# sp-uhh/audio-visual-vad

Hardware: NVIDIA B200
Metric: AV-VAD frames/sec (device-timed) (higher is better)
Workload: dtype bf16

## Files before the change

### audio-visual-vad_b200/csrc/conv_block.cuh

```cuda
#pragma once
#include "conv_slab.cuh"

namespace avvad {
namespace tc {

constexpr int kBlkThreads = 320;
constexpr int kBlkW = 17, kBlkWp = 19;
constexpr int kBlkRows = kBlkWp * kBlkWp;
constexpr uint32_t kBlkSlabBytes = 47104;
constexpr uint32_t kBlkWTile = 32 * 128;
constexpr uint32_t kBlkWBytes = 9 * kBlkWTile;
constexpr uint32_t kBlkOffY = kBlkSlabBytes;
constexpr uint32_t kBlkOffW = 3 * kBlkSlabBytes;
constexpr uint32_t kBlkOffBias = kBlkOffW + 2 * kBlkWBytes;
constexpr uint32_t kBlkOffBar = kBlkOffBias + 512;
constexpr uint32_t kBlkSmem = 1024 + kBlkOffBar + 256;

struct BlockGeom {
  int64_t n_frames;
  int n_pairs;
  const float* bias_a;
  const float* bias_b;
  const __nv_bfloat16* x;
  __nv_bfloat16* z;
};
struct BlockMaps {
  CUtensorMap x;
  CUtensorMap wa;
  CUtensorMap wb;
};

__global__ void __launch_bounds__(kBlkThreads, 1)
tc_block17_kernel(const __grid_constant__ BlockMaps maps, const BlockGeom g) {
  extern __shared__ uint8_t smem_raw[];
  const uint32_t raw = smem_u32(smem_raw);
  const uint32_t base = (raw + 1023u) & ~1023u;
  uint8_t* smem = smem_raw + (base - raw);
  const uint32_t sX = base, sY = base + kBlkOffY, sW = base + kBlkOffW;
  const uint32_t bar0 = base + kBlkOffBar;
  enum { XF = 0, XE, AF, AE, BF, BE, YF0, YF1, YE0, YE1, WF, NBAR };
  auto BAR = [&](int i) { return bar0 + 8u * (uint32_t)i; };
  volatile uint32_t* tmem_slot = reinterpret_cast<volatile uint32_t*>(smem + kBlkOffBar + 8 * (NBAR + 1));
  float* bias_s = reinterpret_cast<float*>(smem + kBlkOffBias);

  const int warp = threadIdx.x >> 5, lane = threadIdx.x & 31;
  const uint32_t rank = pair_rank();
  const int pair = blockIdx.x >> 1;
  const int64_t per_round = 2ll * g.n_pairs;
  const int n_iter = (int)((g.n_frames + per_round - 1) / per_round);

  if (threadIdx.x == 0) {
    mbar_init(BAR(XF), 1);
    mbar_init(BAR(XE), 1);
    mbar_init(BAR(AF), 1);
    mbar_init(BAR(AE), 2 * 8);
    mbar_init(BAR(BF), 1);
    mbar_init(BAR(BE), 2 * 8);
    mbar_init(BAR(YF0), 2 * 8);
    mbar_init(BAR(YF1), 2 * 8);
    mbar_init(BAR(YE0), 1);
    mbar_init(BAR(YE1), 1);
    mbar_init(BAR(WF), 1);
    fence_barrier_init();
    tma_prefetch_desc(&maps.x);
    tma_prefetch_desc(&maps.wa);
    tma_prefetch_desc(&maps.wb);
    mbar_arrive_expect_tx(BAR(WF), 2 * kBlkWBytes);
    for (int tap = 0; tap < 9; ++tap) {
      tma_load_2d(sW + tap * kBlkWTile, &maps.wa, tap * 64, (int)rank * 32, BAR(WF));
      tma_load_2d(sW + kBlkWBytes + tap * kBlkWTile, &maps.wb, tap * 64, (int)rank * 32, BAR(WF));
    }
  }
  if (warp == 1) {
    asm volatile("tcgen05.alloc.cta_group::2.sync.aligned.shared::cta.b32 [%0], %1;" ::"r"(
                     smem_u32(const_cast<uint32_t*>(tmem_slot))),
                 "r"(512)
                 : "memory");
    asm volatile("tcgen05.relinquish_alloc_permit.cta_group::2.sync.aligned;" ::: "memory");
  }
  for (int i = threadIdx.x; i < 128; i += kBlkThreads)
    bias_s[i] = (i < 64) ? (g.bias_a ? g.bias_a[i] : 0.f) : (g.bias_b ? g.bias_b[i - 64] : 0.f);
  for (int i = threadIdx.x; i < 2 * 20 * 8; i += kBlkThreads) {
    const int slab = i / 160, r = i % 160;
    *reinterpret_cast<uint4*>(smem + kBlkOffY + slab * kBlkSlabBytes + r * 16) = make_uint4(0u, 0u, 0u, 0u);
  }
  fence_proxy_async();
  if (warp == 0) mbar_wait(BAR(WF), 0);
  tc_fence_before();
  __syncthreads();
  pair_sync();
  tc_fence_after();
  const uint32_t tmem_acc = *tmem_slot;
  const uint32_t bar0_leader = pair_mapa(bar0, 0);
  auto LBAR = [&](int i) { return bar0_leader + 8u * (uint32_t)i; };

  if (warp == 0) {
    for (int i = 0; i < n_iter; ++i) {
      mbar_wait(BAR(XE), ((uint32_t)i & 1u) ^ 1u);
      if (elect_one_sync()) {
        const int64_t f = ((int64_t)i * g.n_pairs + pair) * 2 + rank;
        if (rank == 0) mbar_arrive_expect_tx(BAR(XF), 2u * kBlkRows * 128u);
        tma_load_4d_2sm(sX, &maps.x, 0, -1, -1, (int)f, LBAR(XF));
      }
      __syncwarp();
    }
  } else if (warp == 1) {
    if (rank == 0) {
      constexpr uint32_t idesc = make_idesc_m256(64);
      auto conv = [&](uint32_t slab, uint32_t wbase, uint32_t d0) {
        const uint32_t slab_lo = desc_lo(slab);
#pragma unroll 1
        for (int tap = 0; tap < 9; ++tap) {
          const uint32_t w_lo = desc_lo(wbase) + (uint32_t)tap * (kBlkWTile >> 4);
          const int fr = tap / 3, fs = tap - fr * 3;
          const uint32_t a0 = slab_lo + (uint32_t)(fr * kBlkWp + fs) * 8u;
#pragma unroll
          for (int m = 0; m < 3; ++m) {
            umma2_f16_lo2(d0 + m * 64, a0 + m * 1024u, w_lo, idesc, tap != 0, kDescHi);
            umma2_f16_lo2(d0 + m * 64, a0 + m * 1024u + 2, w_lo + 2, idesc, 1, kDescHi);
            umma2_f16_lo2(d0 + m * 64, a0 + m * 1024u + 4, w_lo + 4, idesc, 1, kDescHi);
            umma2_f16_lo2(d0 + m * 64, a0 + m * 1024u + 6, w_lo + 6, idesc, 1, kDescHi);
          }
        }
      };
      for (int i = 0; i <= n_iter; ++i) {
        if (i < n_iter) {
          mbar_wait(BAR(XF), (uint32_t)i & 1u);
          mbar_wait(BAR(AE), ((uint32_t)i & 1u) ^ 1u);
          tc_fence_after();
          if (elect_one_sync()) {
            conv(sX, sW, tmem_acc);
            umma2_commit_mc2(BAR(XE));
            umma2_commit_mc2(BAR(AF));
          }
          __syncwarp();
        }
        if (i >= 1) {
          const uint32_t j = (uint32_t)(i - 1), slot = j & 1u;
          mbar_wait(BAR(YF0 + slot), (j >> 1) & 1u);
          mbar_wait(BAR(BE), (j & 1u) ^ 1u);
          tc_fence_after();
          if (elect_one_sync()) {
            conv(sY + slot * kBlkSlabBytes, sW + kBlkWBytes, tmem_acc + 192);
            umma2_commit_mc2(BAR(YE0 + slot));
            umma2_commit_mc2(BAR(BF));
          }
          __syncwarp();
        }
      }
    }
  } else {
    const int q = warp & 3;
    const int jh = (warp - 2) >> 2;
    int loc[3];
    int yrow[3];
#pragma unroll
    for (int m = 0; m < 3; ++m) {
      const int p = m * 128 + q * 32 + lane;
      const int y = p / kBlkWp, x = p - y * kBlkWp;
      loc[m] = (y < kBlkW && x < kBlkW) ? (y * kBlkW + x) * 64 + 32 * jh : -1;
      const int r = p + kBlkWp + 1;
      yrow[m] = (r < kBlkRows) ? r : -1;
    }
    const float* ba = bias_s + 32 * jh;
    const float* bb = bias_s + 64 + 32 * jh;
    const uint32_t lane_sel = (uint32_t)(q * 32) << 16;
    for (int i = 0; i <= n_iter; ++i) {
      if (i < n_iter) {
        const uint32_t slot = (uint32_t)i & 1u;
        mbar_wait(BAR(AF), (uint32_t)i & 1u);
        mbar_wait(BAR(YE0 + slot), (((uint32_t)i >> 1) & 1u) ^ 1u);
        tc_fence_after();
        uint8_t* ys = smem + kBlkOffY + slot * kBlkSlabBytes;
#pragma unroll
        for (int m = 0; m < 3; ++m) {
#pragma unroll
          for (int hc = 0; hc < 2; ++hc) {
            uint32_t v[16];
            tmem_ld16(tmem_acc + (uint32_t)(m * 64 + 32 * jh + 16 * hc) + lane_sel, v);
            tmem_ld_wait();
            if (m == 2 && hc == 1) {
              tc_fence_before();
              __syncwarp();
              if (lane == 0) pair_arrive(LBAR(AE));
            }
            if (yrow[m] >= 0) {
              const bool valid = loc[m] >= 0;
              const int r = yrow[m];
#pragma unroll
              for (int c = 0; c < 2; ++c) {
                uint32_t w[4];
#pragma unroll
                for (int e = 0; e < 4; ++e) {
                  const float f0 = __uint_as_float(v[8 * c + 2 * e]) + ba[16 * hc + 8 * c + 2 * e];
                  const float f1 = __uint_as_float(v[8 * c + 2 * e + 1]) + ba[16 * hc + 8 * c + 2 * e + 1];
                  w[e] = valid ? pack_relu_bf16x2(f0, f1) : 0u;
                }
                const int chunk = (4 * jh + 2 * hc + c) ^ (r & 7);
                *reinterpret_cast<uint4*>(ys + r * 128 + chunk * 16) = make_uint4(w[0], w[1], w[2], w[3]);
              }
            }
          }
        }
        fence_proxy_async();
        __syncwarp();
        if (lane == 0) pair_arrive(LBAR(YF0 + slot));
      }
      if (i >= 1) {
        const int j = i - 1;
        const int64_t f = ((int64_t)j * g.n_pairs + pair) * 2 + rank;
        const bool live = f < g.n_frames;
        const int64_t foff = f * (int64_t)(kBlkW * kBlkW * 64);
        u32x8 rb[3][2] = {};
#pragma unroll
        for (int m = 0; m < 3; ++m)
          if (live && loc[m] >= 0) {
            rb[m][0] = ld_global_256(g.x + foff + loc[m]);
            rb[m][1] = ld_global_256(g.x + foff + loc[m] + 16);
          }
        mbar_wait(BAR(BF), (uint32_t)j & 1u);
        tc_fence_after();
#pragma unroll
        for (int m = 0; m < 3; ++m)
#pragma unroll
          for (int c = 0; c < 2; ++c)
#pragma unroll
            for (int e = 0; e < 8; ++e) asm volatile("" : "+r"(rb[m][c].v[e]));
#pragma unroll
        for (int m = 0; m < 3; ++m) {
#pragma unroll
          for (int c = 0; c < 2; ++c) {
            uint32_t v[16];
            tmem_ld16(tmem_acc + 192u + (uint32_t)(m * 64 + 32 * jh + 16 * c) + lane_sel, v);
            tmem_ld_wait();
            if (m == 2 && c == 1) {
              tc_fence_before();
              __syncwarp();
              if (lane == 0) pair_arrive(LBAR(BE));
            }
            if (live && loc[m] >= 0) {
              u32x8 o;
#pragma unroll
              for (int e = 0; e < 8; ++e) {
                const uint32_t rw = rb[m][c].v[e];
                const float f0 = __uint_as_float(v[2 * e]) + bb[16 * c + 2 * e] + __uint_as_float(rw << 16);
                const float f1 = __uint_as_float(v[2 * e + 1]) + bb[16 * c + 2 * e + 1] + __uint_as_float(rw & 0xFFFF0000u);
                o.v[e] = pack_relu_bf16x2(f0, f1);
              }
              st_global_256(g.z + foff + loc[m] + 16 * c, o);
            }
          }
        }
      }
    }
  }

  tc_fence_before();
  __syncthreads();
  pair_sync();
  if (warp == 1) {
    __syncwarp();
    asm volatile("tcgen05.dealloc.cta_group::2.sync.aligned.b32 %0, %1;" ::"r"(tmem_acc), "r"(512) : "memory");
  }
}

int launch_block17(const __nv_bfloat16* x, const __nv_bfloat16* wa, const float* bias_a, const __nv_bfloat16* wb,
                   const float* bias_b, __nv_bfloat16* z, int64_t n, cudaStream_t st);
bool block17_enabled();

}
}
```

### audio-visual-vad_b200/csrc/conv_slab.cu

```cuda
#include <cudaTypedefs.h>
#include <stdlib.h>

#include <mutex>

#include "conv_slab.cuh"
#include "conv_block.cuh"

namespace avvad {
namespace tc {

int prof_begin(cudaStream_t st, void** tok);
void prof_end(cudaStream_t st, void* tok, int cat, double flops);
int encode_act_map(CUtensorMap* m, const void* ptr, int Cin, int W, int H, int64_t n, const uint32_t box[4],
                   const uint32_t estr[4]);
int encode_weight_map(CUtensorMap* m, const void* ptr, uint64_t K, uint64_t N, uint32_t bn);

bool slab_supported(int H, int W, int Cin, int Cout, int R, int S, int stride, int pad) {
  return tma_available() && R == 3 && S == 3 && stride == 1 && pad == 1 && H == W && Cin == 64 && Cout == 64;
}

struct SlabPlan {
  int F, hb, mb, bn;
  size_t smem;
  double eff;
};

static bool plan(int H, int Cin, int Cout, SlabPlan* out) {
  const int OW = H, OH = H, Wp = OW + 2;
  const int cpb = Cin / 64;
  SlabPlan best{};
  best.eff = -1;
  const int bn = 64;
  for (int hb = 1; hb <= OH; ++hb) {
    const int Hs = hb + 2;
    if (Hs > 256 || Wp > 256) continue;
    const int fmax = (hb == OH) ? 64 : 1;
    for (int F = 1; F <= fmax; ++F) {
      const int rows = F * Hs * Wp;
      const int P = rows - 2 * Wp - 2;
      const int mb = (P + 127) / 128;
      if (2 * mb * bn > 512) break;
      const int slab_rows = mb * 128 + 2 * Wp + 2;
      if (slab_rows < rows) continue;
      const size_t slab_bytes = ((size_t)slab_rows * 128 + 1023) / 1024 * 1024;
      const size_t wbytes = (size_t)9 * cpb * bn * 128;
      const size_t smem = 2 * slab_bytes + wbytes + 256 + 1024 + (size_t)Cout * 4;
      if (smem > 225 * 1024) continue;
      const int nb = (OH + hb - 1) / hb;
      const double eff = (double)OH * OW / ((double)nb * mb * 128.0 / F);
      if (eff > best.eff + 1e-9 || (eff > best.eff - 1e-9 && mb > best.mb)) {
        best.F = F; best.hb = hb; best.mb = mb; best.bn = bn; best.smem = smem; best.eff = eff;
      }
    }
  }
  if (best.eff <= 0) return false;
  *out = best;
  return true;
}

template <int MBC = 0>
static int launch_k(const SlabMaps& maps, const SlabGeom& g, const EpiParams& ep, size_t smem, double flops,
                    cudaStream_t st) {
  static std::mutex mu;
  static size_t attr_set[kMaxDevices] = {};
  {
    int dev = 0;
    AVVAD_CUDA(cudaGetDevice(&dev));
    AVVAD_CHECK_ARG(dev >= 0 && dev < kMaxDevices, "device index out of range");
    std::lock_guard<std::mutex> lk(mu);
    if (smem > attr_set[dev]) {
      AVVAD_CUDA(cudaFuncSetAttribute(tc_slab_kernel<64, MBC>, cudaFuncAttributeMaxDynamicSharedMemorySize, (int)smem));
      attr_set[dev] = smem;
    }
  }
  static int num_sms = [] {
    int dev = 0, n = 148;
    if (cudaGetDevice(&dev) == cudaSuccess) cudaDeviceGetAttribute(&n, cudaDevAttrMultiProcessorCount, dev);
    return n > 0 ? n : 148;
  }();
  void* tok = nullptr;
  const unsigned grid = (unsigned)(g.total_tiles < num_sms ? g.total_tiles : num_sms);
  prof_begin(st, &tok);
  tc_slab_kernel<64, MBC><<<grid, kSlabThreads, smem, st>>>(maps, g, ep);
  AVVAD_LAUNCHED();
  prof_end(st, tok, 0, flops);
  return AVVAD_OK;
}

int launch_slab_conv(const __nv_bfloat16* in, const __nv_bfloat16* w, const EpiParams& ep, int64_t n, int H, int Cin,
                     int Cout, cudaStream_t st) {
  SlabPlan p;
  if (!plan(H, Cin, Cout, &p)) {
    set_error("slab conv: no feasible plan");
    return AVVAD_ERR_ARG;
  }
  SlabGeom g{};
  g.n_frames = n;
  g.OH = H; g.OW = H; g.Wp = H + 2; g.hb = p.hb; g.Hs = p.hb + 2; g.F = p.F; g.mb = p.mb;
  g.nb = (H + p.hb - 1) / p.hb;
  g.cpb = Cin / 64;
  g.N = Cout;
  g.n_tiles = Cout / p.bn;
  g.total_tiles = ((n + p.F - 1) / p.F) * g.nb * g.n_tiles;
  g.slab_rows = p.mb * 128 + 2 * g.Wp + 2;
  g.slab_tx = (uint32_t)p.F * g.Hs * g.Wp * 128u;
  SlabMaps maps;
  const uint32_t box[4] = {64, (uint32_t)g.Wp, (uint32_t)g.Hs, (uint32_t)p.F};
  const uint32_t estr[4] = {1, 1, 1, 1};
  int rc = encode_act_map(&maps.a, in, Cin, H, H, n, box, estr);
  if (rc) return rc;
  rc = encode_weight_map(&maps.b, w, (uint64_t)9 * Cin, (uint64_t)Cout, (uint32_t)p.bn);
  if (rc) return rc;
  const double flops = 2.0 * (double)n * H * H * Cout * 9.0 * Cin;
  if (p.mb == 3) return launch_k<3>(maps, g, ep, p.smem, flops, st);
  return launch_k(maps, g, ep, p.smem, flops, st);
}

bool block17_enabled() {
  static int v = [] {
    const char* e = getenv("AVVAD_BLOCK17");
    return (e && atoi(e) == 0) ? 0 : 1;
  }();
  return v != 0 && tma_available();
}

int launch_block17(const __nv_bfloat16* x, const __nv_bfloat16* wa, const float* bias_a, const __nv_bfloat16* wb,
                   const float* bias_b, __nv_bfloat16* z, int64_t n, cudaStream_t st) {
  AVVAD_CHECK_ARG(x && wa && wb && z && n > 0, "block17: bad argument");
  AVVAD_CHECK_ARG(((reinterpret_cast<uintptr_t>(x) | reinterpret_cast<uintptr_t>(z)) & 31) == 0, "block17: 32-byte aligned activations");
  static PerDeviceOnce once;
  AVVAD_CUDA(once.run([] {
    return cudaFuncSetAttribute(tc_block17_kernel, cudaFuncAttributeMaxDynamicSharedMemorySize, (int)kBlkSmem);
  }));
  static int num_sms = [] {
    int dev = 0, v = 148;
    if (cudaGetDevice(&dev) == cudaSuccess) cudaDeviceGetAttribute(&v, cudaDevAttrMultiProcessorCount, dev);
    return v > 0 ? v : 148;
  }();
  BlockMaps maps;
  const uint32_t box[4] = {64, (uint32_t)kBlkWp, (uint32_t)kBlkWp, 1};
  const uint32_t estr[4] = {1, 1, 1, 1};
  int rc = encode_act_map(&maps.x, x, 64, kBlkW, kBlkW, n, box, estr);
  if (rc) return rc;
  rc = encode_weight_map(&maps.wa, wa, 576, 64, 32);
  if (rc) return rc;
  rc = encode_weight_map(&maps.wb, wb, 576, 64, 32);
  if (rc) return rc;
  BlockGeom g{};
  g.n_frames = n;
  const int64_t want = (n + 1) / 2, pairs = num_sms / 2;
  g.n_pairs = (int)(want < pairs ? want : pairs);
  g.bias_a = bias_a;
  g.bias_b = bias_b;
  g.x = x;
  g.z = z;
  cudaLaunchConfig_t cfg = {};
  cfg.gridDim = dim3(2u * (unsigned)g.n_pairs);
  cfg.blockDim = dim3(kBlkThreads);
  cfg.dynamicSmemBytes = kBlkSmem;
  cfg.stream = st;
  cudaLaunchAttribute la[1];
  la[0].id = cudaLaunchAttributeClusterDimension;
  la[0].val.clusterDim.x = 2; la[0].val.clusterDim.y = 1; la[0].val.clusterDim.z = 1;
  cfg.attrs = la;
  cfg.numAttrs = 1;
  void* tok = nullptr;
  prof_begin(st, &tok);
  cudaError_t le = cudaLaunchKernelEx(&cfg, tc_block17_kernel, maps, g);
  if (le != cudaSuccess) {
    set_error(std::string("block17 launch failed: ") + cudaGetErrorString(le));
    return AVVAD_ERR_CUDA;
  }
  AVVAD_LAUNCHED();
  prof_end(st, tok, 0, 2.0 * 2.0 * (double)n * kBlkW * kBlkW * 64.0 * 576.0);
  return AVVAD_OK;
}

}
}
```

### audio-visual-vad_b200/csrc/gemm_tma.cu

```cuda
#include <cudaTypedefs.h>
#include <stdlib.h>

#include <mutex>

#include "gemm_tma.cuh"

namespace avvad {
namespace tc {

int prof_begin(cudaStream_t st, void** tok);
void prof_end(cudaStream_t st, void* tok, int cat, double flops);

typedef CUresult (*EncodeTiledFn)(CUtensorMap*, CUtensorMapDataType, cuuint32_t, void*, const cuuint64_t*,
                                  const cuuint64_t*, const cuuint32_t*, const cuuint32_t*, CUtensorMapInterleave,
                                  CUtensorMapSwizzle, CUtensorMapL2promotion, CUtensorMapFloatOOBfill);

static EncodeTiledFn encode_fn() {
  static EncodeTiledFn fn = [] {
    void* p = nullptr;
    cudaDriverEntryPointQueryResult q;
    if (cudaGetDriverEntryPoint("cuTensorMapEncodeTiled", &p, cudaEnableDefault, &q) != cudaSuccess ||
        q != cudaDriverEntryPointSuccess)
      p = nullptr;
    return (EncodeTiledFn)p;
  }();
  return fn;
}

bool tma_available() { return encode_fn() != nullptr; }

static int encode4(CUtensorMap* m, const void* ptr, const uint64_t dims[4], const uint64_t strides_bytes[3],
                   const uint32_t box[4], const uint32_t estr[4], bool sw32 = false) {
  EncodeTiledFn fn = encode_fn();
  if (!fn) {
    set_error("cuTensorMapEncodeTiled entry point unavailable");
    return AVVAD_ERR_CUDA;
  }
  cuuint64_t gd[4] = {dims[0], dims[1], dims[2], dims[3]};
  cuuint64_t gs[3] = {strides_bytes[0], strides_bytes[1], strides_bytes[2]};
  cuuint32_t bx[4] = {box[0], box[1], box[2], box[3]};
  cuuint32_t es[4] = {estr[0], estr[1], estr[2], estr[3]};
  CUresult r = fn(m, CU_TENSOR_MAP_DATA_TYPE_BFLOAT16, 4, const_cast<void*>(ptr), gd, gs, bx, es,
                  CU_TENSOR_MAP_INTERLEAVE_NONE, sw32 ? CU_TENSOR_MAP_SWIZZLE_32B : CU_TENSOR_MAP_SWIZZLE_128B,
                  CU_TENSOR_MAP_L2_PROMOTION_L2_128B, CU_TENSOR_MAP_FLOAT_OOB_FILL_NONE);
  if (r != CUDA_SUCCESS) {
    set_error("cuTensorMapEncodeTiled(rank 4) failed with CUresult " + std::to_string((int)r) + " dims=" +
              std::to_string(dims[0]) + "," + std::to_string(dims[1]) + "," + std::to_string(dims[2]) + "," +
              std::to_string(dims[3]) + " box=" + std::to_string(box[0]) + "," + std::to_string(box[1]) + "," +
              std::to_string(box[2]) + "," + std::to_string(box[3]));
    return AVVAD_ERR_CUDA;
  }
  return AVVAD_OK;
}

static int encode2(CUtensorMap* m, const void* ptr, uint64_t inner, uint64_t outer, uint64_t stride_bytes,
                   uint32_t box_inner, uint32_t box_outer, bool sw32 = false) {
  EncodeTiledFn fn = encode_fn();
  if (!fn) {
    set_error("cuTensorMapEncodeTiled entry point unavailable");
    return AVVAD_ERR_CUDA;
  }
  cuuint64_t gd[2] = {inner, outer};
  cuuint64_t gs[1] = {stride_bytes};
  cuuint32_t bx[2] = {box_inner, box_outer};
  cuuint32_t es[2] = {1, 1};
  CUresult r = fn(m, CU_TENSOR_MAP_DATA_TYPE_BFLOAT16, 2, const_cast<void*>(ptr), gd, gs, bx, es,
                  CU_TENSOR_MAP_INTERLEAVE_NONE, sw32 ? CU_TENSOR_MAP_SWIZZLE_32B : CU_TENSOR_MAP_SWIZZLE_128B,
                  CU_TENSOR_MAP_L2_PROMOTION_L2_256B, CU_TENSOR_MAP_FLOAT_OOB_FILL_NONE);
  if (r != CUDA_SUCCESS) {
    set_error("cuTensorMapEncodeTiled(rank 2) failed with CUresult " + std::to_string((int)r));
    return AVVAD_ERR_CUDA;
  }
  return AVVAD_OK;
}

int encode_tiled_bf16(CUtensorMap* m, const void* ptr, int rank, const uint64_t* dims, const uint64_t* strides_bytes,
                      const uint32_t* box) {
  EncodeTiledFn fn = encode_fn();
  if (!fn || rank < 1 || rank > 5) {
    set_error("cuTensorMapEncodeTiled unavailable or bad rank");
    return AVVAD_ERR_CUDA;
  }
  cuuint64_t gd[5], gs[4];
  cuuint32_t bx[5], es[5];
  for (int i = 0; i < rank; ++i) {
    gd[i] = dims[i];
    bx[i] = box[i];
    es[i] = 1;
    if (i < rank - 1) gs[i] = strides_bytes[i];
  }
  CUresult r = fn(m, CU_TENSOR_MAP_DATA_TYPE_BFLOAT16, (cuuint32_t)rank, const_cast<void*>(ptr), gd, gs, bx, es,
                  CU_TENSOR_MAP_INTERLEAVE_NONE, CU_TENSOR_MAP_SWIZZLE_128B, CU_TENSOR_MAP_L2_PROMOTION_L2_128B,
                  CU_TENSOR_MAP_FLOAT_OOB_FILL_NONE);
  if (r != CUDA_SUCCESS) {
    set_error("cuTensorMapEncodeTiled(rank " + std::to_string(rank) + ") failed with CUresult " +
              std::to_string((int)r));
    return AVVAD_ERR_CUDA;
  }
  return AVVAD_OK;
}

int encode_act_map(CUtensorMap* m, const void* ptr, int Cin, int W, int H, int64_t n, const uint32_t box[4],
                   const uint32_t estr[4]) {
  const uint64_t dims[4] = {(uint64_t)Cin, (uint64_t)W, (uint64_t)H, (uint64_t)n};
  const uint64_t strides[3] = {(uint64_t)Cin * 2, (uint64_t)W * Cin * 2, (uint64_t)H * W * Cin * 2};
  return encode4(m, ptr, dims, strides, box, estr);
}
int encode_weight_map(CUtensorMap* m, const void* ptr, uint64_t K, uint64_t N, uint32_t bn) {
  return encode2(m, ptr, K, N, K * 2, 64, bn);
}

static bool pair_enabled() {
  static int v = [] {
    const char* e = getenv("AVVAD_CG2");
    return (e && atoi(e) == 0) ? 0 : 1;
  }();
  return v != 0;
}
static bool use_pair(int bn, int ksplit, int epi_mode, int kb) {
  if (!pair_enabled() || ksplit > 1 || epi_mode == EPI_LSTM) return false;
  return bn == 256 || (bn == 128 && kb >= 16);
}

template <int BN, int KE = 64, int MB = 1, int CG = 1>
static int launch_bn(const TmaMaps& maps, TmaGeom g, const EpiParams& ep, int epi_mode, int cat, double flops,
                     cudaStream_t st) {
  using C = TmaCfg<BN, KE, MB, CG>;
  constexpr int MBT = CG * MB;
  if (g.ksplit < 1) g.ksplit = 1;
  if (g.ksplit == 1) g.kb_split = g.KB;
  g.m_supers = (g.m_tiles + MBT - 1) / MBT;
  g.total_tiles = g.m_supers * g.n_tiles * g.ksplit;
  static PerDeviceOnce once;
  const cudaError_t attr_err = once.run([] {
    return cudaFuncSetAttribute(tc_tma_kernel<BN, KE, MB, CG>, cudaFuncAttributeMaxDynamicSharedMemorySize,
                                (int)C::kSmemBytes);
  });
  if (attr_err != cudaSuccess) {
    set_error(std::string("cudaFuncSetAttribute(smem): ") + cudaGetErrorString(attr_err));
    return AVVAD_ERR_CUDA;
  }
  static int num_sms = [] {
    int dev = 0, n = 148;
    if (cudaGetDevice(&dev) == cudaSuccess) cudaDeviceGetAttribute(&n, cudaDevAttrMultiProcessorCount, dev);
    return n > 0 ? n : 148;
  }();
  if (g.total_tiles <= 0) return AVVAD_OK;
  void* tok = nullptr;
  if (CG == 2) {
    int64_t pairs = num_sms / 2;
    if (g.grid_cap > 0 && g.grid_cap / 2 < pairs) pairs = g.grid_cap / 2 > 0 ? g.grid_cap / 2 : 1;
    cudaLaunchConfig_t cfg = {};
    cfg.gridDim = dim3(2u * (unsigned)(g.total_tiles < pairs ? g.total_tiles : pairs));
    cfg.blockDim = dim3(kTmaThreads);
    cfg.dynamicSmemBytes = C::kSmemBytes;
    cfg.stream = st;
    cudaLaunchAttribute la[1];
    la[0].id = cudaLaunchAttributeClusterDimension;
    la[0].val.clusterDim.x = 2; la[0].val.clusterDim.y = 1; la[0].val.clusterDim.z = 1;
    cfg.attrs = la;
    cfg.numAttrs = 1;
    prof_begin(st, &tok);
    cudaError_t le = cudaLaunchKernelEx(&cfg, tc_tma_kernel<BN, KE, MB, CG>, maps, g, ep, epi_mode);
    if (le != cudaSuccess) {
      set_error(std::string("pair launch failed: ") + cudaGetErrorString(le));
      return AVVAD_ERR_CUDA;
    }
    AVVAD_LAUNCHED();
    prof_end(st, tok, cat, flops);
    return AVVAD_OK;
  }
  int64_t resident = (int64_t)num_sms * C::kCtasPerSm;
  if (g.grid_cap > 0 && g.grid_cap < resident) resident = g.grid_cap;
  const unsigned grid = (unsigned)(g.total_tiles < resident ? g.total_tiles : resident);
  prof_begin(st, &tok);
  tc_tma_kernel<BN, KE, MB, CG><<<grid, kTmaThreads, C::kSmemBytes, st>>>(maps, g, ep, epi_mode);
  AVVAD_LAUNCHED();
  prof_end(st, tok, cat, flops);
  return AVVAD_OK;
}

static int dispatch(int bn, const TmaMaps& maps, const TmaGeom& g, const EpiParams& ep, int epi_mode, int cat,
                    double flops, cudaStream_t st) {
  switch (bn) {
    case 64: return launch_bn<64>(maps, g, ep, epi_mode, cat, flops, st);
    case 128:
      if (g.pair) return launch_bn<128, 64, 2, 2>(maps, g, ep, epi_mode, cat, flops, st);
      if (epi_mode != EPI_LSTM) return launch_bn<128, 64, 2>(maps, g, ep, epi_mode, cat, flops, st);
      return launch_bn<128>(maps, g, ep, epi_mode, cat, flops, st);
    case 256:
      if (g.pair) return launch_bn<256, 64, 1, 2>(maps, g, ep, epi_mode, cat, flops, st);
      return launch_bn<256>(maps, g, ep, epi_mode, cat, flops, st);
  }
  set_error("bad BN");
  return AVVAD_ERR_ARG;
}

static int pick_bn(int N, int hint) {
  if (hint == 64 || hint == 128 || hint == 256) {
    if (N % hint == 0 || hint == 64) return hint;
  }
  if (N <= 64) return 64;
  if (N % 256 == 0) return 256;
  if (N % 128 == 0) return 128;
  return 64;
}

int launch_tma_conv(const __nv_bfloat16* in, const __nv_bfloat16* w, const EpiParams& ep, int64_t n, int H, int W,
                    int Cin, int Cout, int R, int S, int stride, int pad, int bn_hint, cudaStream_t st, int cat,
                    double flops_override, const SecondOperand* second) {
  const int OH = (H + 2 * pad - R) / stride + 1;
  const int OW = (W + 2 * pad - S) / stride + 1;
  const int KE = (Cin % 64 == 0) ? 64 : 16;
  AVVAD_CHECK_ARG(OW <= 128 && Cin % KE == 0, "TMA conv: OW <= 128 and Cin % 64 == 0 (or Cin == 16) required");
  AVVAD_CHECK_ARG(KE == 64 || Cout == 64, "16-channel TMA conv supports Cout == 64 only");
  const bool dual = second && second->in2;
  if (dual) {
    AVVAD_CHECK_ARG(KE == 64 && second->Cin2 % 64 == 0 && second->stride2 >= 1, "second operand: Cin2 % 64 == 0 required");
    AVVAD_CHECK_ARG((second->H2 - 1) / second->stride2 + 1 == OH && (second->W2 - 1) / second->stride2 + 1 == OW,
                    "second operand: output grid mismatch");
  }
  TmaGeom g{};
  g.mode = 1;
  g.OH = OH; g.OW = OW; g.stride = stride; g.pad = pad; g.S = S; g.cpb = Cin / KE; g.KB = R * S * (Cin / KE);
  g.n_frames = n;
  g.N = Cout;
  g.KB2 = dual ? second->Cin2 / 64 : 0;
  g.stride2 = dual ? second->stride2 : 1;
  const int bn = pick_bn(Cout, bn_hint);
  g.n_tiles = (Cout + bn - 1) / bn;
  double best = -1;
  int bh0 = 1, bF0 = 1, bnb0 = OH, brem = 0, bF1 = 1;
  for (int hb0 = 1; hb0 <= OH; ++hb0) {
    if (hb0 * OW > 128) break;
    const int nb0 = OH / hb0;
    const int rem = OH - nb0 * hb0;
    int F0 = (nb0 == 1 && rem == 0) ? 128 / (hb0 * OW) : 128 / (hb0 * OW);
    if (F0 < 1) continue;
    if (nb0 > 1) F0 = 1;
    if (F0 > 256) F0 = 256;
    double tiles_per_frame = (double)nb0 / F0;
    int F1 = 1;
    if (rem > 0) {
      F1 = 128 / (rem * OW);
      if (F1 < 1) continue;
      if (F1 > 256) F1 = 256;
      tiles_per_frame += 1.0 / F1;
    }
    const double eff = (double)OH * OW / (128.0 * tiles_per_frame);
    if (eff > best + 1e-9) {
      best = eff; bh0 = hb0; bF0 = F0; bnb0 = nb0; brem = rem; bF1 = F1;
    }
  }
  AVVAD_CHECK_ARG(best > 0, "TMA conv: no valid tiling");
  g.h0[0] = 0; g.hb[0] = bh0; g.nb[0] = bnb0; g.F[0] = bF0;
  g.tiles0 = ((n + bF0 - 1) / bF0) * bnb0;
  int64_t tiles1 = 0;
  g.h0[1] = bnb0 * bh0; g.hb[1] = brem > 0 ? brem : 1; g.nb[1] = 1; g.F[1] = bF1;
  if (brem > 0) tiles1 = (n + bF1 - 1) / bF1;
  g.m_tiles = g.tiles0 + tiles1;
  g.total_tiles = g.m_tiles * g.n_tiles;

  TmaMaps maps;
  const uint64_t dims[4] = {(uint64_t)Cin, (uint64_t)W, (uint64_t)H, (uint64_t)n};
  const uint64_t strides[3] = {(uint64_t)Cin * 2, (uint64_t)W * Cin * 2, (uint64_t)H * W * Cin * 2};
  const uint32_t estr[4] = {1, (uint32_t)stride, (uint32_t)stride, 1};
  for (int p = 0; p < 2; ++p) {
    const int hb = g.hb[p], F = g.F[p];
    const uint32_t box[4] = {(uint32_t)KE, (uint32_t)((OW - 1) * stride + 1), (uint32_t)((hb - 1) * stride + 1),
                             (uint32_t)F};
    int rc = encode4(&maps.a[p], in, dims, strides, box, estr, KE == 16);
    if (rc) return rc;
    g.bytesA[p] = (uint32_t)F * hb * OW * (uint32_t)(KE * 2);
    if (dual) {
      const int s2 = second->stride2;
      const uint64_t dims2[4] = {(uint64_t)second->Cin2, (uint64_t)second->W2, (uint64_t)second->H2, (uint64_t)n};
      const uint64_t strides2[3] = {(uint64_t)second->Cin2 * 2, (uint64_t)second->W2 * second->Cin2 * 2,
                                    (uint64_t)second->H2 * second->W2 * second->Cin2 * 2};
      const uint32_t estr2[4] = {1, (uint32_t)s2, (uint32_t)s2, 1};
      const uint32_t box2[4] = {64, (uint32_t)((OW - 1) * s2 + 1), (uint32_t)((hb - 1) * s2 + 1), (uint32_t)F};
      rc = encode4(&maps.a2[p], second->in2, dims2, strides2, box2, estr2, false);
      if (rc) return rc;
    } else {
      maps.a2[p] = maps.a[p];
    }
  }
  const int K = R * S * Cin + (dual ? second->Cin2 : 0);
  const bool pair = KE == 64 && use_pair(bn, 1, EPI_BF16, g.KB + g.KB2);
  g.pair = pair ? 1 : 0;
  int rc = encode2(&maps.b, w, (uint64_t)K, (uint64_t)Cout, (uint64_t)K * 2, (uint32_t)KE, (uint32_t)(pair ? bn / 2 : bn),
                   KE == 16);
  if (rc) return rc;
  g.bytesB = (uint32_t)bn * (uint32_t)(KE * 2);
  const double flops = flops_override > 0 ? flops_override : 2.0 * (double)n * OH * OW * Cout * K;
  if (KE == 16) return launch_bn<64, 16>(maps, g, ep, EPI_BF16, cat, flops, st);
  return dispatch(bn, maps, g, ep, EPI_BF16, cat, flops, st);
}

int launch_tma_gemm(const __nv_bfloat16* A, int64_t lda, const __nv_bfloat16* Wt, int64_t ldw, int64_t M, int N, int K,
                    const EpiParams& ep, int epi_mode, int bn_hint, cudaStream_t st, int ksplit, int64_t split_stride) {
  AVVAD_CHECK_ARG(K % 64 == 0 && lda % 8 == 0 && ldw % 8 == 0, "TMA gemm: K % 64, lda % 8, ldw % 8 required");
  AVVAD_CHECK_ARG(ksplit >= 1 && (ksplit == 1 || (epi_mode == EPI_F32 && !ep.bias && !ep.relu)),
                  "split-K needs fp32 output without bias / ReLU");
  TmaGeom g{};
  g.ksplit = ksplit;
  g.kb_split = (K / 64 + ksplit - 1) / ksplit;
  AVVAD_CHECK_ARG((int64_t)(ksplit - 1) * g.kb_split < K / 64, "split-K: empty split (choose ksplit = ceil(KB / ceil(KB / ksplit)))");
  g.split_stride = split_stride;
  g.mode = 0;
  g.KB = K / 64;
  g.cpb = g.KB;
  g.S = 1;
  g.n_frames = M;
  g.N = N;
  int bn = pick_bn(N, bn_hint);
  g.n_tiles = (N + bn - 1) / bn;
  g.m_tiles = (M + BM - 1) / BM;
  g.total_tiles = g.m_tiles * g.n_tiles;
  g.tiles0 = g.m_tiles;
  g.hb[0] = g.hb[1] = 1; g.nb[0] = g.nb[1] = 1; g.F[0] = g.F[1] = 1; g.OW = 128; g.OH = 1;
  TmaMaps maps;
  const uint64_t dims[4] = {(uint64_t)K, (uint64_t)M, 1, 1};
  const uint64_t strides[3] = {(uint64_t)lda * 2, (uint64_t)lda * 2 * (uint64_t)M, (uint64_t)lda * 2 * (uint64_t)M};
  const uint32_t box[4] = {64, 128, 1, 1};
  const uint32_t estr[4] = {1, 1, 1, 1};
  int rc = encode4(&maps.a[0], A, dims, strides, box, estr);
  if (rc) return rc;
  maps.a[1] = maps.a[0];
  maps.a2[0] = maps.a2[1] = maps.a[0];
  g.bytesA[0] = g.bytesA[1] = 128u * 128u;
  g.pair = use_pair(bn, ksplit, epi_mode, g.KB) ? 1 : 0;
  rc = encode2(&maps.b, Wt, (uint64_t)K, (uint64_t)N, (uint64_t)ldw * 2, 64, (uint32_t)(g.pair ? bn / 2 : bn));
  if (rc) return rc;
  g.bytesB = (uint32_t)bn * 128u;
  const double flops = 2.0 * (double)M * N * K;
  return dispatch(bn, maps, g, ep, epi_mode, epi_mode == EPI_LSTM ? 2 : 1, flops, st);
}

int launch_tma_gemm_xt(const __nv_bfloat16* X, int64_t lda, const __nv_bfloat16* Wt, int64_t ldw, int64_t B, int64_t T,
                       int64_t T_stride, int N, int K, const float* bias, float* xT, cudaStream_t st, int grid_cap) {
  AVVAD_CHECK_ARG(K % 64 == 0 && lda % 8 == 0 && ldw % 8 == 0 && N % 32 == 0, "TMA gemm (xT): K % 64, lda % 8, N % 32");
  const int64_t Bp = (B + 127) / 128 * 128;
  AVVAD_CHECK_ARG(T * Bp < (1ll << 31), "TMA gemm (xT): T * B too large");
  TmaGeom g{};
  g.ksplit = 1;
  g.kb_split = K / 64;
  g.mode = 0;
  g.KB = K / 64;
  g.cpb = g.KB;
  g.S = 1;
  g.n_frames = T * Bp;
  g.N = N;
  g.tm_bp = (int)Bp;
  g.tm_b = (int)B;
  g.grid_cap = grid_cap;
  const int bn = pick_bn(N, 0);
  g.n_tiles = (N + bn - 1) / bn;
  g.m_tiles = T * Bp / BM;
  g.total_tiles = g.m_tiles * g.n_tiles;
  g.tiles0 = g.m_tiles;
  g.hb[0] = g.hb[1] = 1; g.nb[0] = g.nb[1] = 1; g.F[0] = g.F[1] = 1; g.OW = 128; g.OH = 1;
  TmaMaps maps;
  const uint64_t dims[4] = {(uint64_t)K, (uint64_t)B, (uint64_t)T, 1};
  const uint64_t strides[3] = {(uint64_t)lda * 2 * (uint64_t)T_stride, (uint64_t)lda * 2,
                               (uint64_t)lda * 2 * (uint64_t)T_stride * (uint64_t)B};
  const uint32_t box[4] = {64, 128, 1, 1};
  const uint32_t estr[4] = {1, 1, 1, 1};
  int rc = encode4(&maps.a[0], X, dims, strides, box, estr);
  if (rc) return rc;
  maps.a[1] = maps.a[0];
  maps.a2[0] = maps.a2[1] = maps.a[0];
  g.bytesA[0] = g.bytesA[1] = 128u * 128u;
  g.pair = use_pair(bn, 1, EPI_XT, g.KB) ? 1 : 0;
  rc = encode2(&maps.b, Wt, (uint64_t)K, (uint64_t)N, (uint64_t)ldw * 2, 64, (uint32_t)(g.pair ? bn / 2 : bn));
  if (rc) return rc;
  g.bytesB = (uint32_t)bn * 128u;
  EpiParams ep{};
  ep.bias = bias;
  ep.C = xT;
  ep.ldc = N;
  return dispatch(bn, maps, g, ep, EPI_XT, 1, 2.0 * (double)B * T * N * K, st);
}

int launch_tma_gemm_tm(const __nv_bfloat16* X, int64_t lda, const __nv_bfloat16* Wt, int64_t ldw, int64_t B, int64_t T,
                       int64_t T_stride, int N, int K, float* C, int64_t ldc, cudaStream_t st, int grid_cap) {
  AVVAD_CHECK_ARG(K % 64 == 0 && lda % 8 == 0 && ldw % 8 == 0 && N % 32 == 0, "TMA gemm (tm): K % 64, lda % 8, N % 32");
  const int64_t Bp = (B + 127) / 128 * 128;
  AVVAD_CHECK_ARG(T * Bp < (1ll << 31), "TMA gemm (xT): T * B too large");
  TmaGeom g{};
  g.ksplit = 1;
  g.kb_split = K / 64;
  g.mode = 0;
  g.KB = K / 64;
  g.cpb = g.KB;
  g.S = 1;
  g.n_frames = T * Bp;
  g.N = N;
  g.tm_bp = (int)Bp;
  g.tm_b = (int)B;
  g.tm_tstride = T_stride;
  g.grid_cap = grid_cap;
  const int bn = pick_bn(N, 0);
  g.n_tiles = (N + bn - 1) / bn;
  g.m_tiles = T * Bp / BM;
  g.total_tiles = g.m_tiles * g.n_tiles;
  g.tiles0 = g.m_tiles;
  g.hb[0] = g.hb[1] = 1; g.nb[0] = g.nb[1] = 1; g.F[0] = g.F[1] = 1; g.OW = 128; g.OH = 1;
  TmaMaps maps;
  const uint64_t dims[4] = {(uint64_t)K, (uint64_t)B, (uint64_t)T, 1};
  const uint64_t strides[3] = {(uint64_t)lda * 2 * (uint64_t)T_stride, (uint64_t)lda * 2,
                               (uint64_t)lda * 2 * (uint64_t)T_stride * (uint64_t)B};
  const uint32_t box[4] = {64, 128, 1, 1};
  const uint32_t estr[4] = {1, 1, 1, 1};
  int rc = encode4(&maps.a[0], X, dims, strides, box, estr);
  if (rc) return rc;
  maps.a[1] = maps.a[0];
  maps.a2[0] = maps.a2[1] = maps.a[0];
  g.bytesA[0] = g.bytesA[1] = 128u * 128u;
  g.pair = use_pair(bn, 1, EPI_F32, g.KB) ? 1 : 0;
  rc = encode2(&maps.b, Wt, (uint64_t)K, (uint64_t)N, (uint64_t)ldw * 2, 64, (uint32_t)(g.pair ? bn / 2 : bn));
  if (rc) return rc;
  g.bytesB = (uint32_t)bn * 128u;
  EpiParams ep{};
  ep.C = C;
  ep.ldc = ldc;
  return dispatch(bn, maps, g, ep, EPI_F32, 1, 2.0 * (double)B * T * N * K, st);
}


}
}
```

### audio-visual-vad_b200/csrc/gemm_tma.cuh

```cuda
#pragma once
#include <cuda.h>

#include "gemm_tc.cuh"

namespace avvad {
namespace tc {

constexpr int kTmaThreads = 320;
constexpr int kTmaEpiWarps = 8;
template <int BN>
struct TmaBias {
  static constexpr int kEntries = (BN == 256) ? 4096 : 1024;
};

struct TmaGeom {
  int mode;
  int n_tiles;
  int64_t total_tiles;
  int64_t m_tiles;
  int64_t tiles0;
  int h0[2], hb[2], nb[2], F[2];
  int OH, OW, stride, pad, S, cpb, KB;
  int KB2, stride2;
  int ksplit, kb_split;
  int64_t split_stride, m_supers;
  int64_t n_frames;
  int N;
  int tm_bp, tm_b;
  int64_t tm_tstride;
  int pair;
  int grid_cap;
  uint32_t bytesA[2];
  uint32_t bytesB;
};

struct TmaMaps {
  CUtensorMap a[2];
  CUtensorMap a2[2];
  CUtensorMap b;
};

__device__ __forceinline__ void mbar_arrive_expect_tx(uint32_t bar, uint32_t bytes) {
  asm volatile("mbarrier.arrive.expect_tx.shared::cta.b64 _, [%0], %1;" ::"r"(bar), "r"(bytes) : "memory");
}
__device__ __forceinline__ void tma_load_4d(uint32_t dst, const CUtensorMap* map, int c0, int c1, int c2, int c3,
                                            uint32_t bar) {
  asm volatile(
      "cp.async.bulk.tensor.4d.shared::cluster.global.tile.mbarrier::complete_tx::bytes [%0], [%1, {%2, %3, %4, %5}], [%6];"
      ::"r"(dst), "l"(map), "r"(c0), "r"(c1), "r"(c2), "r"(c3), "r"(bar)
      : "memory");
}
__device__ __forceinline__ void tma_load_2d(uint32_t dst, const CUtensorMap* map, int c0, int c1, uint32_t bar) {
  asm volatile(
      "cp.async.bulk.tensor.2d.shared::cluster.global.tile.mbarrier::complete_tx::bytes [%0], [%1, {%2, %3}], [%4];"
      ::"r"(dst), "l"(map), "r"(c0), "r"(c1), "r"(bar)
      : "memory");
}
__device__ __forceinline__ void umma_f16_lo2(uint32_t tmem_d, uint32_t a_lo, uint32_t b_lo, uint32_t idesc,
                                             uint32_t accum, uint32_t hi) {
  asm volatile(
      "{\n\t.reg .pred p;\n\t.reg .b64 da, db;\n\t"
      "mov.b64 da, {%1, %5};\n\t"
      "mov.b64 db, {%2, %5};\n\t"
      "setp.ne.b32 p, %4, 0;\n\t"
      "tcgen05.mma.cta_group::1.kind::f16 [%0], da, db, %3, p;\n\t}"
      ::"r"(tmem_d), "r"(a_lo), "r"(b_lo), "r"(idesc), "r"(accum), "r"(hi)
      : "memory");
}
__device__ __forceinline__ void tma_load_4d_2sm(uint32_t dst, const CUtensorMap* map, int c0, int c1, int c2, int c3,
                                                uint32_t bar_leader) {
  asm volatile(
      "cp.async.bulk.tensor.4d.cta_group::2.shared::cluster.global.tile.mbarrier::complete_tx::bytes "
      "[%0], [%1, {%2, %3, %4, %5}], [%6];"
      ::"r"(dst), "l"(map), "r"(c0), "r"(c1), "r"(c2), "r"(c3), "r"(bar_leader)
      : "memory");
}
__device__ __forceinline__ void tma_load_2d_2sm(uint32_t dst, const CUtensorMap* map, int c0, int c1, uint32_t bar_leader) {
  asm volatile(
      "cp.async.bulk.tensor.2d.cta_group::2.shared::cluster.global.tile.mbarrier::complete_tx::bytes "
      "[%0], [%1, {%2, %3}], [%4];"
      ::"r"(dst), "l"(map), "r"(c0), "r"(c1), "r"(bar_leader)
      : "memory");
}
__device__ __forceinline__ void umma2_f16_lo2(uint32_t tmem_d, uint32_t a_lo, uint32_t b_lo, uint32_t idesc,
                                              uint32_t accum, uint32_t hi) {
  asm volatile(
      "{\n\t.reg .pred p;\n\t.reg .b64 da, db;\n\t"
      "mov.b64 da, {%1, %5};\n\t"
      "mov.b64 db, {%2, %5};\n\t"
      "setp.ne.b32 p, %4, 0;\n\t"
      "tcgen05.mma.cta_group::2.kind::f16 [%0], da, db, %3, p;\n\t}"
      ::"r"(tmem_d), "r"(a_lo), "r"(b_lo), "r"(idesc), "r"(accum), "r"(hi)
      : "memory");
}
__device__ __forceinline__ void umma2_commit_mc2(uint32_t bar) {
  asm volatile(
      "tcgen05.commit.cta_group::2.mbarrier::arrive::one.shared::cluster.multicast::cluster.b64 [%0], %1;"
      ::"r"(bar), "h"((uint16_t)3)
      : "memory");
}
__device__ __forceinline__ uint32_t pair_rank() {
  uint32_t r;
  asm volatile("mov.u32 %0, %%cluster_ctarank;" : "=r"(r));
  return r;
}
__device__ __forceinline__ uint32_t pair_mapa(uint32_t addr, uint32_t rank) {
  uint32_t r;
  asm volatile("mapa.shared::cluster.u32 %0, %1, %2;" : "=r"(r) : "r"(addr), "r"(rank));
  return r;
}
__device__ __forceinline__ void pair_arrive(uint32_t cluster_addr) {
  asm volatile("mbarrier.arrive.release.cluster.shared::cluster.b64 _, [%0];" ::"r"(cluster_addr) : "memory");
}
__device__ __forceinline__ void pair_sync() {
  asm volatile("barrier.cluster.arrive.release.aligned;" ::: "memory");
  asm volatile("barrier.cluster.wait.acquire.aligned;" ::: "memory");
}
__host__ __device__ constexpr uint32_t make_idesc_m256(int n) {
  return (1u << 4) | (1u << 7) | (1u << 10) | ((uint32_t)(n >> 3) << 17) | ((uint32_t)(256 >> 4) << 24);
}
__device__ __forceinline__ void tma_prefetch_desc(const CUtensorMap* map) {
  asm volatile("prefetch.tensormap [%0];" ::"l"(map) : "memory");
}

template <int BN, int KE = 64, int MB = 1, int CG = 1>
struct TmaCfg {
  static constexpr uint32_t kRowBytes = KE * 2;
  static constexpr uint32_t kABytes = BM * kRowBytes;
  static constexpr uint32_t kBBytes = (BN / CG) * kRowBytes;
  static constexpr uint32_t kStageBytes = MB * kABytes + kBBytes;
  static constexpr int kCtasPerSm = (BN == 256 || MB > 1 || CG == 2) ? 1 : 2;
  static constexpr int kStages =
      (CG == 2) ? (int)((200u * 1024u) / kStageBytes)
                : ((KE == 16) ? 8 : ((BN == 256) ? 4 : ((BN == 128) ? (MB > 1 ? 4 : 3) : 4)));
  static_assert(CG == 1 || (KE == 64 && (BN == 256 || BN == 128)), "pair mode: BN = 256 or 128");
  static constexpr uint32_t kSmemBytes = kStages * kStageBytes + 1024 + 256 + TmaBias<BN>::kEntries * 4;
  static constexpr uint32_t kDescHiWord = ((8 * kRowBytes) >> 4) | (1u << 14) | ((KE == 64 ? 2u : 6u) << 29);
  static_assert(2 * MB * BN <= 512, "TMEM: two accumulator stages of MB x BN columns");
};

struct TileCoord {
  int phase;
  int64_t n0;
  int hstart;
  bool valid;
};

__device__ __forceinline__ TileCoord decode_block(const TmaGeom& g, int64_t mt) {
  TileCoord t;
  t.valid = mt < g.m_tiles;
  if (!t.valid) mt = g.m_tiles - 1;
  if (g.mode == 0) {
    t.phase = 0;
    t.n0 = mt * BM;
    t.hstart = 0;
    return t;
  }
  t.phase = (mt < g.tiles0) ? 0 : 1;
  if (t.phase) mt -= g.tiles0;
  const int nb = g.nb[t.phase];
  const int band = (int)(mt % nb);
  t.n0 = (mt / nb) * g.F[t.phase];
  t.hstart = g.h0[t.phase] + band * g.hb[t.phase];
  return t;
}

template <int BN, int KE, int MB, int CG = 1>
__global__ void __launch_bounds__(kTmaThreads, TmaCfg<BN, KE, MB, CG>::kCtasPerSm)
tc_tma_kernel(const __grid_constant__ TmaMaps maps, const __grid_constant__ TmaGeom g, const EpiParams ep,
              const int epi_mode) {
  using C = TmaCfg<BN, KE, MB, CG>;
  constexpr int S = C::kStages;
  constexpr int MBT = CG * MB;
  const uint32_t rank = (CG == 2) ? pair_rank() : 0u;
  const int64_t tile0 = (CG == 2) ? (int64_t)(blockIdx.x >> 1) : (int64_t)blockIdx.x;
  const int64_t tile_step = (CG == 2) ? (int64_t)(gridDim.x >> 1) : (int64_t)gridDim.x;
  constexpr uint32_t kAccCols = MB * BN;
  constexpr uint32_t kTmemCols = 2 * kAccCols;
  extern __shared__ uint8_t smem_raw[];
  const uint32_t raw = smem_u32(smem_raw);
  const uint32_t base = (raw + 1023u) & ~1023u;
  uint8_t* smem = smem_raw + (base - raw);
  const uint32_t bar0 = base + S * C::kStageBytes;
  volatile uint32_t* tmem_slot = reinterpret_cast<volatile uint32_t*>(smem + S * C::kStageBytes + 8 * (2 * S + 4));

  const int warp = threadIdx.x >> 5;
  const int lane = threadIdx.x & 31;

  if (threadIdx.x == 0) {
    for (int s = 0; s < S; ++s) {
      mbar_init(bar0 + 8 * s, 1);
      mbar_init(bar0 + 8 * (S + s), 1);
    }
    for (int a = 0; a < 2; ++a) {
      mbar_init(bar0 + 8 * (2 * S + a), 1);
      mbar_init(bar0 + 8 * (2 * S + 2 + a), CG * kTmaEpiWarps);
    }
    fence_barrier_init();
    tma_prefetch_desc(&maps.a[0]);
    tma_prefetch_desc(&maps.a[1]);
    if (g.KB2 > 0) {
      tma_prefetch_desc(&maps.a2[0]);
      tma_prefetch_desc(&maps.a2[1]);
    }
    tma_prefetch_desc(&maps.b);
  }
  float* bias_s = reinterpret_cast<float*>(smem + S * C::kStageBytes + 256);
  const bool bias_in_smem = g.N <= TmaBias<BN>::kEntries;
  if (bias_in_smem)
    for (int i = threadIdx.x; i < g.N; i += kTmaThreads) bias_s[i] = ep.bias ? ep.bias[i] : 0.f;
  if (warp == 1) {
    if (CG == 2) {
      asm volatile("tcgen05.alloc.cta_group::2.sync.aligned.shared::cta.b32 [%0], %1;" ::"r"(
                       smem_u32(const_cast<uint32_t*>(tmem_slot))),
                   "r"(kTmemCols)
                   : "memory");
      asm volatile("tcgen05.relinquish_alloc_permit.cta_group::2.sync.aligned;" ::: "memory");
    } else {
      tmem_alloc(smem_u32(const_cast<uint32_t*>(tmem_slot)), kTmemCols);
      tmem_relinquish();
    }
  }
  tc_fence_before();
  __syncthreads();
  if (CG == 2) pair_sync();
  tc_fence_after();
  const uint32_t tmem_acc = *tmem_slot;
  const uint32_t bar0_leader = (CG == 2) ? pair_mapa(bar0, 0) : bar0;

  if (warp == 0) {
    uint32_t it = 0;
    for (int64_t tile = tile0; tile < g.total_tiles; tile += tile_step) {
      const int n_base = (int)(tile % g.n_tiles) * BN + (int)rank * (BN / CG);
      const int64_t sm = (tile / g.n_tiles) % g.m_supers;
      const int split = (int)(tile / (g.n_tiles * g.m_supers));
      const int kb0 = split * g.kb_split;
      const int kb1 = (kb0 + g.kb_split < g.KB) ? kb0 + g.kb_split : g.KB;
      TileCoord t[MB];
      uint32_t bytes = g.bytesB;
#pragma unroll
      for (int mb = 0; mb < MB; ++mb) {
        t[mb] = decode_block(g, sm * MBT + mb + (CG == 2 ? (int)rank * MB : 0));
        bytes += g.bytesA[t[mb].phase];
      }
      if (CG == 2) {
#pragma unroll
        for (int mb = 0; mb < MB; ++mb) bytes += g.bytesA[decode_block(g, sm * MBT + mb + (1 - (int)rank) * MB).phase];
      }
      int cb = 0, fr = 0, fs = 0;
      for (int kb = kb0; kb < kb1; ++kb, ++it) {
        const int s = it % S;
        const uint32_t ph = (it / S) & 1u;
        mbar_wait(bar0 + 8 * (S + s), ph ^ 1u);
        if (elect_one_sync()) {
          const uint32_t sa = base + s * C::kStageBytes;
          if (CG == 2) {
            const uint32_t full = bar0_leader + 8 * s;
            if (rank == 0) mbar_arrive_expect_tx(bar0 + 8 * s, bytes);
#pragma unroll
            for (int mb = 0; mb < MB; ++mb) {
              const uint32_t da = sa + mb * C::kABytes;
              if (g.mode == 0) {
                if (g.tm_bp)
                  tma_load_4d_2sm(da, &maps.a[0], kb * KE, (int)(t[mb].n0 % g.tm_bp), (int)(t[mb].n0 / g.tm_bp), 0, full);
                else
                  tma_load_4d_2sm(da, &maps.a[0], kb * KE, (int)t[mb].n0, 0, 0, full);
              } else {
                tma_load_4d_2sm(da, &maps.a[t[mb].phase], cb * KE, fs - g.pad, t[mb].hstart * g.stride + fr - g.pad,
                                (int)t[mb].n0, full);
              }
            }
            tma_load_2d_2sm(sa + MB * C::kABytes, &maps.b, kb * KE, n_base, full);
          } else {
          const uint32_t full = bar0 + 8 * s;
          mbar_arrive_expect_tx(full, bytes);
#pragma unroll
          for (int mb = 0; mb < MB; ++mb) {
            if (g.mode == 0) {
              if (g.tm_bp)
                tma_load_4d(sa + mb * C::kABytes, &maps.a[0], kb * KE, (int)(t[mb].n0 % g.tm_bp),
                            (int)(t[mb].n0 / g.tm_bp), 0, full);
              else
                tma_load_4d(sa + mb * C::kABytes, &maps.a[0], kb * KE, (int)t[mb].n0, 0, 0, full);
            } else {
              tma_load_4d(sa + mb * C::kABytes, &maps.a[t[mb].phase], cb * KE, fs - g.pad,
                          t[mb].hstart * g.stride + fr - g.pad, (int)t[mb].n0, full);
            }
          }
          tma_load_2d(sa + MB * C::kABytes, &maps.b, kb * KE, n_base, full);
          }
        }
        __syncwarp();
        if (++cb == g.cpb) {
          cb = 0;
          if (++fs == g.S) {
            fs = 0;
            ++fr;
          }
        }
      }
      for (int kb2 = 0; kb2 < g.KB2; ++kb2, ++it) {
        const int s = it % S;
        const uint32_t ph = (it / S) & 1u;
        mbar_wait(bar0 + 8 * (S + s), ph ^ 1u);
        if (elect_one_sync()) {
          const uint32_t sa = base + s * C::kStageBytes;
          if (CG == 2) {
            const uint32_t full = bar0_leader + 8 * s;
            if (rank == 0) mbar_arrive_expect_tx(bar0 + 8 * s, bytes);
#pragma unroll
            for (int mb = 0; mb < MB; ++mb)
              tma_load_4d_2sm(sa + mb * C::kABytes, &maps.a2[t[mb].phase], kb2 * KE, 0, t[mb].hstart * g.stride2,
                              (int)t[mb].n0, full);
            tma_load_2d_2sm(sa + MB * C::kABytes, &maps.b, (g.KB + kb2) * KE, n_base, full);
          } else {
          const uint32_t full = bar0 + 8 * s;
          mbar_arrive_expect_tx(full, bytes);
#pragma unroll
          for (int mb = 0; mb < MB; ++mb)
            tma_load_4d(sa + mb * C::kABytes, &maps.a2[t[mb].phase], kb2 * KE, 0, t[mb].hstart * g.stride2,
                        (int)t[mb].n0, full);
          tma_load_2d(sa + MB * C::kABytes, &maps.b, (g.KB + kb2) * KE, n_base, full);
          }
        }
        __syncwarp();
      }
    }
  } else if (warp == 1) {
    constexpr uint32_t idesc = (CG == 2) ? make_idesc_m256(BN) : make_idesc(BN);
    uint32_t it = 0, tl = 0;
    if (CG == 1 || rank == 0)
    for (int64_t tile = tile0; tile < g.total_tiles; tile += tile_step, ++tl) {
      const uint32_t acc = tl & 1u, aph = (tl >> 1) & 1u;
      const int split = (int)(tile / (g.n_tiles * g.m_supers));
      const int kbs = split * g.kb_split;
      const int kb_total = ((kbs + g.kb_split < g.KB) ? g.kb_split : g.KB - kbs) + g.KB2;
      mbar_wait(bar0 + 8 * (2 * S + 2 + acc), aph ^ 1u);
      tc_fence_after();
      const uint32_t d_tmem = tmem_acc + acc * kAccCols;
      for (int kb = 0; kb < kb_total; ++kb, ++it) {
        const int s = it % S;
        const uint32_t ph = (it / S) & 1u;
        mbar_wait(bar0 + 8 * s, ph);
        tc_fence_after();
        if (elect_one_sync()) {
          const uint32_t a0 = desc_lo(base + s * C::kStageBytes);
          const uint32_t b_lo = a0 + ((MB * C::kABytes) >> 4);
#pragma unroll
          for (int mb = 0; mb < MB; ++mb) {
            const uint32_t a_lo = a0 + ((mb * C::kABytes) >> 4);
            const uint32_t d = d_tmem + mb * BN;
            if (CG == 2) {
              umma2_f16_lo2(d, a_lo, b_lo, idesc, kb != 0, C::kDescHiWord);
              umma2_f16_lo2(d, a_lo + 2, b_lo + 2, idesc, 1, C::kDescHiWord);
              umma2_f16_lo2(d, a_lo + 4, b_lo + 4, idesc, 1, C::kDescHiWord);
              umma2_f16_lo2(d, a_lo + 6, b_lo + 6, idesc, 1, C::kDescHiWord);
              continue;
            }
            umma_f16_lo2(d, a_lo, b_lo, idesc, kb != 0, C::kDescHiWord);
            if (KE == 64) {
              umma_f16_lo2(d, a_lo + 2, b_lo + 2, idesc, 1, C::kDescHiWord);
              umma_f16_lo2(d, a_lo + 4, b_lo + 4, idesc, 1, C::kDescHiWord);
              umma_f16_lo2(d, a_lo + 6, b_lo + 6, idesc, 1, C::kDescHiWord);
            }
          }
          if (CG == 2) {
            umma2_commit_mc2(bar0 + 8 * (S + s));
            if (kb == kb_total - 1) umma2_commit_mc2(bar0 + 8 * (2 * S + acc));
          } else {
            umma_commit(bar0 + 8 * (S + s));
            if (kb == kb_total - 1) umma_commit(bar0 + 8 * (2 * S + acc));
          }
        }
        __syncwarp();
      }
    }
  } else {
    const int q = warp & 3;
    const int half = (warp - 2) >> 2;
    constexpr int kJ = BN / 32;
    constexpr int kMine = (kJ + 1) / 2;
    const bool fast = (epi_mode == EPI_BF16) && bias_in_smem && (g.N % 32 == 0);
    const bool fast32 = (epi_mode == EPI_F32) && bias_in_smem && (g.N % 32 == 0) && (ep.ldc % 4 == 0) &&
                        ((reinterpret_cast<uintptr_t>(ep.C) & 15) == 0);
    uint32_t tl = 0;
    for (int64_t tile = tile0; tile < g.total_tiles; tile += tile_step, ++tl) {
      const int n_base = (int)(tile % g.n_tiles) * BN;
      const int64_t sm = (tile / g.n_tiles) % g.m_supers;
      const int64_t c_off = (tile / (g.n_tiles * g.m_supers)) * g.split_stride;
      const uint32_t acc = tl & 1u, aph = (tl >> 1) & 1u;
      const int r = q * 32 + lane;
      int64_t m[MB];
#pragma unroll
      for (int mb = 0; mb < MB; ++mb) {
        const TileCoord t = decode_block(g, sm * MBT + mb + (CG == 2 ? (int)rank * MB : 0));
        m[mb] = -1;
        if (!t.valid) continue;
        if (g.mode == 0) {
          if (t.n0 + r < g.n_frames) m[mb] = t.n0 + r;
          if (g.tm_bp && epi_mode != EPI_XT && m[mb] >= 0) {
            const int64_t tt = m[mb] / g.tm_bp, bb = m[mb] - tt * g.tm_bp;
            m[mb] = (bb < g.tm_b) ? bb * g.tm_tstride + tt : -1;
          }
        } else {
          const int hb = g.hb[t.phase];
          const int per_frame = hb * g.OW;
          const int f = r / per_frame;
          const int rem = r - f * per_frame;
          const int hh = rem / g.OW;
          const int ww = rem - hh * g.OW;
          const int oh = t.hstart + hh;
          if (f < g.F[t.phase] && t.n0 + f < g.n_frames && oh < g.OH)
            m[mb] = ((t.n0 + f) * g.OH + oh) * g.OW + ww;
        }
      }
      const uint32_t t_row = tmem_acc + acc * kAccCols + ((uint32_t)(q * 32) << 16);
      if (fast) {
        u32x8 rb[MB * kMine][2] = {};
        const bool wide = ((reinterpret_cast<uintptr_t>(ep.C) | reinterpret_cast<uintptr_t>(ep.residual)) & 31) == 0 &&
                          (ep.ldc % 16 == 0);
        if (ep.residual) {
#pragma unroll
          for (int mb = 0; mb < MB; ++mb)
#pragma unroll
            for (int i = 0; i < kMine; ++i) {
              const int n0 = n_base + (2 * i + half) * 32;
              if (m[mb] >= 0 && 2 * i + half < kJ && n0 < g.N) {
                const __nv_bfloat16* rp = ep.residual + m[mb] * ep.ldc + n0;
                if (wide) {
                  rb[mb * kMine + i][0] = ld_global_256(rp);
                  rb[mb * kMine + i][1] = ld_global_256(rp + 16);
                } else {
                  const uint4* r4 = reinterpret_cast<const uint4*>(rp);
#pragma unroll
                  for (int c = 0; c < 4; ++c) {
                    const uint4 t4 = r4[c];
                    rb[mb * kMine + i][c >> 1].v[4 * (c & 1) + 0] = t4.x;
                    rb[mb * kMine + i][c >> 1].v[4 * (c & 1) + 1] = t4.y;
                    rb[mb * kMine + i][c >> 1].v[4 * (c & 1) + 2] = t4.z;
                    rb[mb * kMine + i][c >> 1].v[4 * (c & 1) + 3] = t4.w;
                  }
                }
              }
            }
        }
        mbar_wait(bar0 + 8 * (2 * S + acc), aph);
        tc_fence_after();
#pragma unroll
        for (int i = 0; i < MB * kMine; ++i)
#pragma unroll
          for (int c = 0; c < 2; ++c)
#pragma unroll
            for (int e = 0; e < 8; ++e) asm volatile("" : "+r"(rb[i][c].v[e]));
#pragma unroll
        for (int mb = 0; mb < MB; ++mb)
#pragma unroll
          for (int i = 0; i < kMine; ++i) {
            const int j = 2 * i + half;
            if (j < kJ) {
              uint32_t v[32];
              tmem_ld32(t_row + mb * BN + j * 32, v);
              tmem_ld_wait();
              const int n0 = n_base + j * 32;
              if (m[mb] >= 0 && n0 < g.N) {
                float f32[32];
                const float4* bp = reinterpret_cast<const float4*>(bias_s + n0);
#pragma unroll
                for (int c = 0; c < 8; ++c) {
                  const float4 b4 = bp[c];
                  f32[4 * c + 0] = __uint_as_float(v[4 * c + 0]) + b4.x;
                  f32[4 * c + 1] = __uint_as_float(v[4 * c + 1]) + b4.y;
                  f32[4 * c + 2] = __uint_as_float(v[4 * c + 2]) + b4.z;
                  f32[4 * c + 3] = __uint_as_float(v[4 * c + 3]) + b4.w;
                }
                if (ep.residual) {
#pragma unroll
                  for (int e = 0; e < 16; ++e) {
                    const uint32_t w = rb[mb * kMine + i][e >> 3].v[e & 7];
                    f32[2 * e + 0] += __uint_as_float(w << 16);
                    f32[2 * e + 1] += __uint_as_float(w & 0xFFFF0000u);
                  }
                }
                __nv_bfloat16* cp = reinterpret_cast<__nv_bfloat16*>(ep.C) + m[mb] * ep.ldc + n0;
#pragma unroll
                for (int c = 0; c < 2; ++c) {
                  u32x8 o;
#pragma unroll
                  for (int e = 0; e < 8; ++e)
                    o.v[e] = ep.relu ? pack_relu_bf16x2(f32[16 * c + 2 * e], f32[16 * c + 2 * e + 1])
                                     : pack_bf16x2(f32[16 * c + 2 * e], f32[16 * c + 2 * e + 1]);
                  if (wide) {
                    st_global_256(cp + 16 * c, o);
                  } else {
                    uint4* c4 = reinterpret_cast<uint4*>(cp + 16 * c);
                    c4[0] = make_uint4(o.v[0], o.v[1], o.v[2], o.v[3]);
                    c4[1] = make_uint4(o.v[4], o.v[5], o.v[6], o.v[7]);
                  }
                }
              }
            }
          }
      } else if (epi_mode == EPI_XT) {
        mbar_wait(bar0 + 8 * (2 * S + acc), aph);
        tc_fence_after();
        const int U = g.N >> 2;
#pragma unroll
        for (int mb = 0; mb < MB; ++mb) {
          const int tt = (m[mb] >= 0) ? (int)(m[mb] / g.tm_bp) : 0;
          const int bb = (m[mb] >= 0) ? (int)(m[mb] - (int64_t)tt * g.tm_bp) : g.tm_b;
#pragma unroll 1
          for (int j = half; j < kJ; j += 2) {
            uint32_t v[32];
            tmem_ld32(t_row + mb * BN + j * 32, v);
            tmem_ld_wait();
            const int n0 = n_base + j * 32;
            if (bb < g.tm_b && n0 < g.N) {
              float4* dst = reinterpret_cast<float4*>(ep.C) + ((int64_t)tt * U + (n0 >> 2)) * g.tm_bp + bb;
#pragma unroll
              for (int c = 0; c < 8; ++c) {
                float4 b4;
                if (bias_in_smem) b4 = reinterpret_cast<const float4*>(bias_s + n0)[c];
                else b4 = ep.bias ? __ldg(reinterpret_cast<const float4*>(ep.bias + n0) + c) : make_float4(0.f, 0.f, 0.f, 0.f);
                dst[(int64_t)c * g.tm_bp] = make_float4(__uint_as_float(v[4 * c + 0]) + b4.x, __uint_as_float(v[4 * c + 1]) + b4.y,
                                                        __uint_as_float(v[4 * c + 2]) + b4.z, __uint_as_float(v[4 * c + 3]) + b4.w);
              }
            }
          }
        }
      } else if (fast32) {
        mbar_wait(bar0 + 8 * (2 * S + acc), aph);
        tc_fence_after();
#pragma unroll
        for (int mb = 0; mb < MB; ++mb) {
#pragma unroll 1
          for (int j = half; j < kJ; j += 2) {
            uint32_t v[32];
            tmem_ld32(t_row + mb * BN + j * 32, v);
            tmem_ld_wait();
            const int n0 = n_base + j * 32;
            if (m[mb] >= 0 && n0 < g.N) {
              const float4* bp = reinterpret_cast<const float4*>(bias_s + n0);
              float* crow = reinterpret_cast<float*>(ep.C) + c_off + m[mb] * ep.ldc + n0;
              const bool wide32 = (reinterpret_cast<uintptr_t>(crow) & 31) == 0;
#pragma unroll
              for (int c = 0; c < 4; ++c) {
                const float4 ba = bp[2 * c], bb = bp[2 * c + 1];
                float o[8] = {__uint_as_float(v[8 * c + 0]) + ba.x, __uint_as_float(v[8 * c + 1]) + ba.y,
                              __uint_as_float(v[8 * c + 2]) + ba.z, __uint_as_float(v[8 * c + 3]) + ba.w,
                              __uint_as_float(v[8 * c + 4]) + bb.x, __uint_as_float(v[8 * c + 5]) + bb.y,
                              __uint_as_float(v[8 * c + 6]) + bb.z, __uint_as_float(v[8 * c + 7]) + bb.w};
                if (ep.relu) {
#pragma unroll
                  for (int e = 0; e < 8; ++e) o[e] = fmaxf(o[e], 0.f);
                }
                if (wide32) {
                  u32x8 w;
#pragma unroll
                  for (int e = 0; e < 8; ++e) w.v[e] = __float_as_uint(o[e]);
                  st_global_256(crow + 8 * c, w);
                } else {
                  reinterpret_cast<float4*>(crow + 8 * c)[0] = make_float4(o[0], o[1], o[2], o[3]);
                  reinterpret_cast<float4*>(crow + 8 * c)[1] = make_float4(o[4], o[5], o[6], o[7]);
                }
              }
            }
          }
        }
      } else {
        mbar_wait(bar0 + 8 * (2 * S + acc), aph);
        tc_fence_after();
#pragma unroll
        for (int mb = 0; mb < MB; ++mb) {
#pragma unroll 1
          for (int j = half; j < kJ; j += 2) {
            uint32_t v[32];
            tmem_ld32(t_row + mb * BN + j * 32, v);
            tmem_ld_wait();
            const int n0 = n_base + j * 32;
            if (m[mb] >= 0 && n0 < g.N) {
              EpiParams e2 = ep;
              if (epi_mode == EPI_F32) e2.C = reinterpret_cast<float*>(ep.C) + c_off;
              epilogue_chunk(e2, epi_mode, v, m[mb], n0, g.N);
            }
          }
        }
      }
      tc_fence_before();
      __syncwarp();
      if (lane == 0) {
        if (CG == 2) pair_arrive(bar0_leader + 8 * (2 * S + 2 + acc));
        else mbar_arrive(bar0 + 8 * (2 * S + 2 + acc));
      }
    }
  }

  tc_fence_before();
  __syncthreads();
  if (CG == 2) pair_sync();
  if (warp == 1) {
    __syncwarp();
    if (CG == 2) asm volatile("tcgen05.dealloc.cta_group::2.sync.aligned.b32 %0, %1;" ::"r"(tmem_acc), "r"(kTmemCols) : "memory");
    else tmem_dealloc(tmem_acc, kTmemCols);
  }
}

bool tma_available();
struct SecondOperand {
  const __nv_bfloat16* in2 = nullptr;
  int H2 = 0, W2 = 0, Cin2 = 0, stride2 = 1;
};
int launch_tma_conv(const __nv_bfloat16* in, const __nv_bfloat16* w, const EpiParams& ep, int64_t n, int H, int W,
                    int Cin, int Cout, int R, int S, int stride, int pad, int bn_hint, cudaStream_t st, int cat = 0,
                    double flops_override = 0.0, const SecondOperand* second = nullptr);
int launch_tma_gemm(const __nv_bfloat16* A, int64_t lda, const __nv_bfloat16* Wt, int64_t ldw, int64_t M, int N, int K,
                    const EpiParams& ep, int epi_mode, int bn_hint, cudaStream_t st, int ksplit = 1,
                    int64_t split_stride = 0);
int launch_tma_gemm_xt(const __nv_bfloat16* X, int64_t lda, const __nv_bfloat16* Wt, int64_t ldw, int64_t B, int64_t T,
                       int64_t T_stride, int N, int K, const float* bias, float* xT, cudaStream_t st, int grid_cap = 0);
int launch_tma_gemm_tm(const __nv_bfloat16* X, int64_t lda, const __nv_bfloat16* Wt, int64_t ldw, int64_t B, int64_t T,
                       int64_t T_stride, int N, int K, float* C, int64_t ldc, cudaStream_t st, int grid_cap = 0);

}
}
```

### audio-visual-vad_b200/csrc/resnet.cu

```cuda
#include <stdlib.h>

#include <mutex>

#include "gemm_tma.cuh"
#include "stem_s2d.cuh"

namespace avvad {
namespace tc {
int launch_block17(const __nv_bfloat16* x, const __nv_bfloat16* wa, const float* bias_a, const __nv_bfloat16* wb,
                   const float* bias_b, __nv_bfloat16* z, int64_t n, cudaStream_t st);
bool block17_enabled();
}
}

namespace avvad {

struct ConvSpec {
  int cin, cout, k, stride, pad, hin, hout;
};
static const ConvSpec kSpecs[20] = {
    {3, 64, 7, 2, 3, 67, 34},
    {64, 64, 3, 1, 1, 17, 17},   {64, 64, 3, 1, 1, 17, 17},
    {64, 64, 3, 1, 1, 17, 17},   {64, 64, 3, 1, 1, 17, 17},
    {64, 128, 3, 2, 1, 17, 9},   {128, 128, 3, 1, 1, 9, 9},  {64, 128, 1, 2, 0, 17, 9},
    {128, 128, 3, 1, 1, 9, 9},   {128, 128, 3, 1, 1, 9, 9},
    {128, 256, 3, 2, 1, 9, 5},   {256, 256, 3, 1, 1, 5, 5},  {128, 256, 1, 2, 0, 9, 5},
    {256, 256, 3, 1, 1, 5, 5},   {256, 256, 3, 1, 1, 5, 5},
    {256, 512, 3, 2, 1, 5, 3},   {512, 512, 3, 1, 1, 3, 3},  {256, 512, 1, 2, 0, 5, 3},
    {512, 512, 3, 1, 1, 3, 3},   {512, 512, 3, 1, 1, 3, 3},
};
constexpr int64_t kFrameHW = 67 * 67;
constexpr int64_t kActBytesPerFrame = 17 * 17 * 64 * 2;

__global__ void pack_conv_kernel(const float* __restrict__ w, const float* __restrict__ gamma,
                                 const float* __restrict__ beta, const float* __restrict__ mean,
                                 const float* __restrict__ var, float eps, int cout, int cin, int k,
                                 __nv_bfloat16* __restrict__ wp, float* __restrict__ bias) {
  const int idx = blockIdx.x * blockDim.x + threadIdx.x;
  const int total = cout * cin * k * k;
  if (idx < cout) {
    const float sc = gamma[idx] / sqrtf(var[idx] + eps);
    bias[idx] = beta[idx] - mean[idx] * sc;
  }
  if (idx >= total) return;
  const int i = idx % cin;
  const int s = (idx / cin) % k;
  const int r = (idx / (cin * k)) % k;
  const int o = idx / (cin * k * k);
  const float sc = gamma[o] / sqrtf(var[o] + eps);
  wp[idx] = __float2bfloat16_rn(w[((o * cin + i) * k + r) * k + s] * sc);
}

__global__ void pack_conv1_tc_kernel(const float* __restrict__ w, const float* __restrict__ gamma,
                                     const float* __restrict__ beta, const float* __restrict__ mean,
                                     const float* __restrict__ var, float eps, __nv_bfloat16* __restrict__ w1b,
                                     float* __restrict__ bias) {
  const int idx = blockIdx.x * blockDim.x + threadIdx.x;
  if (idx < 64) {
    const float sc = gamma[idx] / sqrtf(var[idx] + eps);
    bias[idx] = beta[idx] - mean[idx] * sc;
  }
  if (idx >= 64 * 64) return;
  const int o = idx / 64, k = idx % 64;
  float v = 0.f;
  if (k < 49) {
    const float sc = gamma[o] / sqrtf(var[o] + eps);
    v = (w[(o * 3 + 0) * 49 + k] + w[(o * 3 + 1) * 49 + k] + w[(o * 3 + 2) * 49 + k]) * sc;
  }
  w1b[idx] = __float2bfloat16_rn(v);
}

__global__ void concat_ds_kernel(const __nv_bfloat16* __restrict__ wb, const __nv_bfloat16* __restrict__ wds,
                                 const float* __restrict__ bb, const float* __restrict__ bds, int cout, int kb, int kds,
                                 __nv_bfloat16* __restrict__ wf, float* __restrict__ bf) {
  const int idx = blockIdx.x * blockDim.x + threadIdx.x;
  const int kt = kb + kds;
  if (idx < cout) bf[idx] = bb[idx] + bds[idx];
  if (idx >= cout * kt) return;
  const int o = idx / kt, k = idx - o * kt;
  wf[idx] = (k < kb) ? wb[o * kb + k] : wds[o * kds + (k - kb)];
}

__global__ void avgpool_kernel(const __nv_bfloat16* __restrict__ act, int64_t n_frames, int hw, int C,
                               float* __restrict__ feat, __nv_bfloat16* __restrict__ feat_bf16, int64_t ld_bf16,
                               int64_t col_off) {
  const int64_t idx = (int64_t)blockIdx.x * blockDim.x + threadIdx.x;
  const int chunks = C / 8;
  if (idx >= n_frames * chunks) return;
  const int64_t f = idx / chunks;
  const int ch = (int)(idx - f * chunks);
  float s[8] = {0, 0, 0, 0, 0, 0, 0, 0};
  const __nv_bfloat16* p = act + f * hw * C + ch * 8;
  for (int i = 0; i < hw; ++i) {
    const uint4 v = *reinterpret_cast<const uint4*>(p + (int64_t)i * C);
    const float2 a = unpack_bf16x2(v.x), b = unpack_bf16x2(v.y), c = unpack_bf16x2(v.z), d = unpack_bf16x2(v.w);
    s[0] += a.x; s[1] += a.y; s[2] += b.x; s[3] += b.y; s[4] += c.x; s[5] += c.y; s[6] += d.x; s[7] += d.y;
  }
  const float inv = 1.0f / (float)hw;
#pragma unroll
  for (int q = 0; q < 8; ++q) s[q] *= inv;
  if (feat) {
    float4* o = reinterpret_cast<float4*>(feat + f * C + ch * 8);
    o[0] = make_float4(s[0], s[1], s[2], s[3]);
    o[1] = make_float4(s[4], s[5], s[6], s[7]);
  }
  if (feat_bf16) {
    __nv_bfloat16* o = feat_bf16 + f * ld_bf16 + col_off + ch * 8;
#pragma unroll
    for (int q = 0; q < 8; ++q) o[q] = __float2bfloat16_rn(s[q]);
  }
}

constexpr int kStatRows = 2048;
__global__ void __launch_bounds__(256) bn_stats_kernel(const __nv_bfloat16* __restrict__ raw, int64_t M, int C,
                                                       double* __restrict__ stats) {
  extern __shared__ float st_sm[];
  const int groups = C / 8;
  const int lanes = 256 / groups;
  const int gidx = threadIdx.x % groups, ln = threadIdx.x / groups;
  const int64_t r0 = (int64_t)blockIdx.x * kStatRows;
  const int64_t r1 = (r0 + kStatRows < M) ? r0 + kStatRows : M;
  float s[8] = {0, 0, 0, 0, 0, 0, 0, 0}, q[8] = {0, 0, 0, 0, 0, 0, 0, 0};
  for (int64_t r = r0 + ln; r < r1; r += lanes) {
    const uint4 v = *reinterpret_cast<const uint4*>(raw + r * C + gidx * 8);
    const uint32_t w[4] = {v.x, v.y, v.z, v.w};
#pragma unroll
    for (int e = 0; e < 4; ++e) {
      const float a = __uint_as_float(w[e] << 16), b = __uint_as_float(w[e] & 0xFFFF0000u);
      s[2 * e] += a; q[2 * e] = fmaf(a, a, q[2 * e]);
      s[2 * e + 1] += b; q[2 * e + 1] = fmaf(b, b, q[2 * e + 1]);
    }
  }
  float* mine = st_sm + (size_t)ln * 2 * C + gidx * 8;
#pragma unroll
  for (int e = 0; e < 8; ++e) {
    mine[e] = s[e];
    mine[C + e] = q[e];
  }
  __syncthreads();
  for (int c = threadIdx.x; c < 2 * C; c += 256) {
    double acc = 0.0;
    for (int l = 0; l < lanes; ++l) acc += (double)st_sm[(size_t)l * 2 * C + c];
    atomicAdd(stats + c, acc);
  }
}
__global__ void bn_finalize_kernel(const double* __restrict__ stats, int64_t M, int C, float eps, float momentum,
                                   const float* __restrict__ gamma, const float* __restrict__ beta,
                                   float* __restrict__ scale_shift, float* __restrict__ running_mean,
                                   float* __restrict__ running_var, float* __restrict__ mean_invstd_out = nullptr) {
  const int c = blockIdx.x * blockDim.x + threadIdx.x;
  if (c >= C) return;
  const double mean = stats[c] / (double)M;
  double var = stats[C + c] / (double)M - mean * mean;
  if (var < 0) var = 0;
  if (mean_invstd_out) {
    mean_invstd_out[c] = (float)mean;
    mean_invstd_out[C + c] = (float)(1.0 / sqrt(var + (double)eps));
  }
  const double a = (1.0 / sqrt(var + (double)eps)) * (double)gamma[c];
  scale_shift[c] = (float)a;
  scale_shift[C + c] = (float)((double)beta[c] - mean * a);
  if (running_mean) {
    const double unbiased = M > 1 ? var * (double)M / (double)(M - 1) : var;
    running_mean[c] = (1.f - momentum) * running_mean[c] + momentum * (float)mean;
    running_var[c] = (1.f - momentum) * running_var[c] + momentum * (float)unbiased;
  }
}
constexpr int kApplyRows = 4;
__global__ void __launch_bounds__(256) bn_apply_kernel(const __nv_bfloat16* __restrict__ raw, int64_t M, int C,
                                                       const float* __restrict__ scale_shift,
                                                       const __nv_bfloat16* __restrict__ residual, int relu,
                                                       __nv_bfloat16* __restrict__ out) {
  extern __shared__ float ss_sm[];
  for (int i = threadIdx.x; i < 2 * C; i += 256) ss_sm[i] = scale_shift[i];
  __syncthreads();
  const int groups = C / 8;
  const int rows_per_block = (256 / groups) * kApplyRows;
  const int gidx = threadIdx.x % groups, ln = threadIdx.x / groups;
  float a[8], b[8];
#pragma unroll
  for (int e = 0; e < 8; ++e) {
    a[e] = ss_sm[gidx * 8 + e];
    b[e] = ss_sm[C + gidx * 8 + e];
  }
  const int64_t base = (int64_t)blockIdx.x * rows_per_block + ln;
  uint4 v[kApplyRows], rv[kApplyRows];
#pragma unroll
  for (int k = 0; k < kApplyRows; ++k) {
    const int64_t r = base + (int64_t)k * (256 / groups);
    if (r < M) {
      v[k] = *reinterpret_cast<const uint4*>(raw + r * C + gidx * 8);
      if (residual) rv[k] = *reinterpret_cast<const uint4*>(residual + r * C + gidx * 8);
    }
  }
#pragma unroll
  for (int k = 0; k < kApplyRows; ++k) {
    const int64_t r = base + (int64_t)k * (256 / groups);
    if (r >= M) continue;
    const uint32_t w[4] = {v[k].x, v[k].y, v[k].z, v[k].w};
    const uint32_t rw[4] = {rv[k].x, rv[k].y, rv[k].z, rv[k].w};
    uint32_t o[4];
#pragma unroll
    for (int e = 0; e < 4; ++e) {
      float y0 = fmaf(__uint_as_float(w[e] << 16), a[2 * e], b[2 * e]);
      float y1 = fmaf(__uint_as_float(w[e] & 0xFFFF0000u), a[2 * e + 1], b[2 * e + 1]);
      if (residual) {
        y0 += __uint_as_float(rw[e] << 16);
        y1 += __uint_as_float(rw[e] & 0xFFFF0000u);
      }
      o[e] = relu ? pack_relu_bf16x2(y0, y1) : pack_bf16x2(y0, y1);
    }
    *reinterpret_cast<uint4*>(out + r * C + gidx * 8) = make_uint4(o[0], o[1], o[2], o[3]);
  }
}
__global__ void pack_conv_raw_kernel(const float* __restrict__ w, int cout, int cin, int k,
                                     __nv_bfloat16* __restrict__ wp) {
  const int idx = blockIdx.x * blockDim.x + threadIdx.x;
  if (idx >= cout * cin * k * k) return;
  const int i = idx % cin;
  const int s = (idx / cin) % k;
  const int r = (idx / (cin * k)) % k;
  const int o = idx / (cin * k * k);
  wp[idx] = __float2bfloat16_rn(w[((o * cin + i) * k + r) * k + s]);
}
__global__ void pack_conv1_raw32_kernel(const float* __restrict__ w, float* __restrict__ w32) {
  const int idx = blockIdx.x * blockDim.x + threadIdx.x;
  if (idx >= 64 * 49) return;
  const int o = idx / 49, k = idx % 49;
  w32[idx] = w[(o * 3 + 0) * 49 + k] + w[(o * 3 + 1) * 49 + k] + w[(o * 3 + 2) * 49 + k];
}
__global__ void fold_conv1_kernel(const float* __restrict__ w32, const float* __restrict__ scale_shift,
                                  __nv_bfloat16* __restrict__ w1fold) {
  const int idx = blockIdx.x * blockDim.x + threadIdx.x;
  if (idx >= 64 * 64) return;
  const int o = idx / 64, k = idx % 64;
  w1fold[idx] = __float2bfloat16_rn(k < 49 ? w32[o * 49 + k] * scale_shift[o] : 0.f);
}
__global__ void pack_conv1_raw_kernel(const float* __restrict__ w, __nv_bfloat16* __restrict__ w1) {
  const int idx = blockIdx.x * blockDim.x + threadIdx.x;
  if (idx >= 64 * 64) return;
  const int o = idx / 64, k = idx % 64;
  float v = 0.f;
  if (k < 49) v = w[(o * 3 + 0) * 49 + k] + w[(o * 3 + 1) * 49 + k] + w[(o * 3 + 2) * 49 + k];
  w1[idx] = __float2bfloat16_rn(v);
}

}

using namespace avvad;

struct avvad_resnet18 {
  __nv_bfloat16* w[20];
  float* bias[20];
  __nv_bfloat16* w1b;
  bool set[20];
  __nv_bfloat16* wf[3];
  float* bf[3];
  bool fused_ready;
  __nv_bfloat16* wraw[20];
  float* w1raw32;
  __nv_bfloat16* w1fold;
  float* gamma[20];
  float* beta[20];
  bool set_train[20];
};

extern "C" int avvad_resnet18_create(avvad_resnet18** out) {
  AVVAD_CHECK_ARG(out, "null out");
  avvad_resnet18* h = new avvad_resnet18();
  for (int i = 0; i < 20; ++i) {
    h->w[i] = nullptr;
    h->bias[i] = nullptr;
    h->set[i] = false;
  }
  for (int i = 0; i < 20; ++i) {
    h->wraw[i] = nullptr;
    h->gamma[i] = h->beta[i] = nullptr;
    h->set_train[i] = false;
  }
  h->w1b = nullptr;
  for (int i = 0; i < 3; ++i) {
    h->wf[i] = nullptr;
    h->bf[i] = nullptr;
  }
  h->fused_ready = false;
  h->w1raw32 = nullptr;
  h->w1fold = nullptr;
  for (int i = 0; i < 20; ++i) {
    const ConvSpec& s = kSpecs[i];
    AVVAD_CUDA(cudaMalloc(&h->bias[i], sizeof(float) * s.cout));
    if (i == 0) {
      AVVAD_CUDA(cudaMalloc(&h->w1b, sizeof(__nv_bfloat16) * 64 * 64));
    } else {
      AVVAD_CUDA(cudaMalloc(&h->w[i], sizeof(__nv_bfloat16) * (size_t)s.cout * s.cin * s.k * s.k));
    }
  }
  *out = h;
  return AVVAD_OK;
}

extern "C" void avvad_resnet18_destroy(avvad_resnet18* h) {
  if (!h) return;
  for (int i = 0; i < 20; ++i) {
    cudaFree(h->w[i]);
    cudaFree(h->bias[i]);
  }
  for (int i = 0; i < 20; ++i) {
    cudaFree(h->wraw[i]);
    cudaFree(h->gamma[i]);
    cudaFree(h->beta[i]);
  }
  cudaFree(h->w1b);
  cudaFree(h->w1raw32);
  cudaFree(h->w1fold);
  for (int i = 0; i < 3; ++i) {
    cudaFree(h->wf[i]);
    cudaFree(h->bf[i]);
  }
  delete h;
}

extern "C" int avvad_resnet18_set_conv(avvad_resnet18* h, int layer, const float* w, const float* gamma,
                                       const float* beta, const float* mean, const float* var, float bn_eps,
                                       void* stream) {
  AVVAD_CHECK_ARG(h && layer >= 0 && layer < 20, "bad handle/layer");
  AVVAD_CHECK_ARG(w && gamma && beta && mean && var, "null pointer");
  cudaStream_t st = (cudaStream_t)stream;
  const ConvSpec& s = kSpecs[layer];
  if (layer == 0) {
    pack_conv1_tc_kernel<<<(64 * 64 + 255) / 256, 256, 0, st>>>(w, gamma, beta, mean, var, bn_eps, h->w1b, h->bias[0]);
  } else {
    const int total = s.cout * s.cin * s.k * s.k;
    pack_conv_kernel<<<(total + 255) / 256, 256, 0, st>>>(w, gamma, beta, mean, var, bn_eps, s.cout, s.cin, s.k,
                                                          h->w[layer], h->bias[layer]);
  }
  AVVAD_LAUNCHED();
  h->set[layer] = true;
  h->fused_ready = false;
  return AVVAD_OK;
}

static const int kDsBlocks[3][2] = {{6, 7}, {11, 12}, {16, 17}};

static int build_fused(avvad_resnet18* h, cudaStream_t st) {
  if (h->fused_ready) return AVVAD_OK;
  for (int i = 0; i < 3; ++i) {
    const int lb = kDsBlocks[i][0], lds = kDsBlocks[i][1];
    const ConvSpec& sb = kSpecs[lb];
    const ConvSpec& sd = kSpecs[lds];
    const int kb = sb.k * sb.k * sb.cin, kds = sd.cin;
    const size_t total = (size_t)sb.cout * (kb + kds);
    if (!h->wf[i]) {
      AVVAD_CUDA(cudaMalloc(&h->wf[i], total * sizeof(__nv_bfloat16)));
      AVVAD_CUDA(cudaMalloc(&h->bf[i], sb.cout * sizeof(float)));
    }
    concat_ds_kernel<<<(unsigned)ceil_div((int64_t)total, 256), 256, 0, st>>>(h->w[lb], h->w[lds], h->bias[lb],
                                                                             h->bias[lds], sb.cout, kb, kds, h->wf[i],
                                                                             h->bf[i]);
    AVVAD_LAUNCHED();
  }
  h->fused_ready = true;
  return AVVAD_OK;
}

static int64_t chunk_of(int64_t n_frames, int64_t chunk) {
  if (chunk <= 0) chunk = 2048;
  return n_frames < chunk ? n_frames : chunk;
}

extern "C" size_t avvad_resnet18_workspace_bytes(int64_t n_frames, int64_t chunk_frames) {
  if (n_frames <= 0) return 0;
  const int64_t mc = chunk_of(n_frames, chunk_frames);
  return (size_t)(4 * align_up((size_t)mc * kActBytesPerFrame, 1024));
}

static int run_conv(avvad_resnet18* h, int layer, const __nv_bfloat16* in, const __nv_bfloat16* residual,
                    __nv_bfloat16* out, int64_t n, int relu, cudaStream_t st) {
  const ConvSpec& s = kSpecs[layer];
  return avvad_conv2d_nhwc_bf16(in, h->w[layer], h->bias[layer], residual, out, n, s.hin, s.hin, s.cin, s.cout, s.k,
                                s.k, s.stride, s.pad, relu, st);
}

struct StemInput {
  const float* frames = nullptr;
  const uint8_t* src = nullptr;
  const int32_t* n_src = nullptr;
  const int32_t* n_out = nullptr;
  int f_max = 0, t_max = 0, num = 0, den = 0, standardise = 0;
  int64_t src_bytes = 0;
  float mean = 0.f, denom = 1.f;
  StemInput advance(int64_t f0) const {
    StemInput r = *this;
    r.first = first + f0;
    return r;
  }
  int64_t first = 0;
};

static int launch_stem_s2d(avvad_resnet18* h, const StemInput& in, int64_t n, __nv_bfloat16* out, cudaStream_t st,
                           const __nv_bfloat16* w = nullptr, const float* bias = nullptr, double* stats = nullptr) {
  static PerDeviceOnce once;
  AVVAD_CUDA(once.run([] {
    cudaError_t e = cudaFuncSetAttribute(tc::stem_s2d_kernel<0>, cudaFuncAttributeMaxDynamicSharedMemorySize, (int)tc::kS2Smem);
    if (e == cudaSuccess)
      e = cudaFuncSetAttribute(tc::stem_s2d_kernel<1>, cudaFuncAttributeMaxDynamicSharedMemorySize, (int)tc::kS2Smem);
    if (e == cudaSuccess)
      e = cudaFuncSetAttribute(tc::stem_s2d_kernel<0, true>, cudaFuncAttributeMaxDynamicSharedMemorySize, (int)tc::kS2Smem);
    return e;
  }));
  static int num_sms = [] {
    int dev = 0, v = 148;
    if (cudaGetDevice(&dev) == cudaSuccess) cudaDeviceGetAttribute(&v, cudaDevAttrMultiProcessorCount, dev);
    return v > 0 ? v : 148;
  }();
  tc::StemS2Params p{};
  p.n_frames = n;
  p.w1b = w ? w : h->w1b;
  p.bias = w ? bias : h->bias[0];
  p.out = out;
  p.stats = stats;
  const int64_t batches = (n + tc::kS2FramesPerBatch - 1) / tc::kS2FramesPerBatch;
  const unsigned grid = (unsigned)(batches < num_sms ? batches : num_sms);
  void* tok = nullptr;
  tc::prof_begin(st, &tok);
  if (in.src) {
    p.src = in.src; p.n_src = in.n_src; p.n_out = in.n_out; p.src_bytes = in.src_bytes;
    p.f_max = in.f_max; p.t_max = in.t_max; p.num = in.num; p.den = in.den;
    p.mean = in.mean; p.denom = in.denom; p.standardise = in.standardise;
    p.first = in.first;
    tc::stem_s2d_kernel<1><<<grid, tc::kS2Threads, tc::kS2Smem, st>>>(p);
  } else if (stats) {
    p.frames = in.frames + in.first * kFrameHW;
    tc::stem_s2d_kernel<0, true><<<grid, tc::kS2Threads, tc::kS2Smem, st>>>(p);
  } else {
    p.frames = in.frames + in.first * kFrameHW;
    tc::stem_s2d_kernel<0><<<grid, tc::kS2Threads, tc::kS2Smem, st>>>(p);
  }
  AVVAD_LAUNCHED();
  tc::prof_end(st, tok, 3, 2.0 * (double)n * 1156 * 64 * 49);
  return AVVAD_OK;
}

static int launch_stem(avvad_resnet18* h, const StemInput& in, int64_t n, __nv_bfloat16* out, cudaStream_t st) {
  return launch_stem_s2d(h, in, n, out, st);
}

static const int64_t kStageIn[4] = {17 * 17 * 64, 17 * 17 * 64, 9 * 9 * 128, 5 * 5 * 256};
static const int64_t kStageOut[4] = {17 * 17 * 64, 9 * 9 * 128, 5 * 5 * 256, 3 * 3 * 512};
static const double kStageMac[4] = {42614784.0, 42467328.0, 52428800.0, 75497472.0};

static int run_trunk_chunk(avvad_resnet18* h, const StemInput& in, int64_t n, __nv_bfloat16* const buf[4], int upto,
                           int* last, cudaStream_t st) {
  int frc = build_fused(h, st);
  if (frc) return frc;
  const bool whole = upto < 20;
  int cur = 0;
  *last = cur;
  int layer = 1;
  for (int stage = 0; stage < 4; ++stage) {
    {
      const int64_t f0 = 0, nn = n;
      if (stage == 0) {
        int rc = launch_stem(h, in.advance(f0), nn, buf[0] + f0 * kStageIn[0], st);
        if (rc) return rc;
        if (upto == 0) return AVVAD_OK;
      }
      void* gtok = nullptr;
      if (!whole) tc::prof_group_begin(st, &gtok);
      struct GroupEnd {
        cudaStream_t st; void* tok; double flops;
        ~GroupEnd() { tc::prof_group_end(st, tok, 0, flops); }
      } group_end{st, gtok, 2.0 * (double)nn * kStageMac[stage]};
      for (int blk = 0; blk < 2; ++blk) {
        int o[3], k = 0;
        for (int i = 0; i < 4; ++i)
          if (i != cur) o[k++] = i;
        const bool ds = (stage > 0 && blk == 0);
        const int la = layer, lb = layer + 1, lds = layer + 2;
        const __nv_bfloat16* xin = buf[cur] + f0 * (blk == 0 ? kStageIn[stage] : kStageOut[stage]);
        __nv_bfloat16* y0 = buf[o[0]] + f0 * kStageOut[stage];
        __nv_bfloat16* y1 = buf[o[1]] + f0 * kStageOut[stage];
        __nv_bfloat16* y2 = buf[o[2]] + f0 * kStageOut[stage];
        if (stage == 0 && !whole && tc::block17_enabled() &&
            ((reinterpret_cast<uintptr_t>(xin) | reinterpret_cast<uintptr_t>(y2)) & 31) == 0) {
          int rcb = tc::launch_block17(xin, h->w[la], h->bias[la], h->w[lb], h->bias[lb], y2, nn, st);
          if (rcb) return rcb;
          cur = o[2];
          *last = cur;
          layer += 2;
          continue;
        }
        int rc = run_conv(h, la, xin, nullptr, y0, nn, 1, st);
        if (rc) return rc;
        if (upto == la) { *last = o[0]; return AVVAD_OK; }
        const __nv_bfloat16* res = xin;
        if (ds && upto != lds) {
          const ConvSpec& sb = kSpecs[lb];
          const ConvSpec& sd = kSpecs[lds];
          tc::EpiParams ep{};
          ep.bias = h->bf[stage - 1];
          ep.C = y2;
          ep.ldc = sb.cout;
          ep.relu = 1;
          tc::SecondOperand so;
          so.in2 = xin;
          so.H2 = sd.hin; so.W2 = sd.hin; so.Cin2 = sd.cin; so.stride2 = sd.stride;
          rc = tc::launch_tma_conv(y0, h->wf[stage - 1], ep, nn, sb.hin, sb.hin, sb.cin, sb.cout, sb.k, sb.k, sb.stride,
                                   sb.pad, 0, st, 0, 0.0, &so);
          if (rc) return rc;
          cur = o[2];
          *last = cur;
          if (upto == lb) return AVVAD_OK;
          layer += 3;
          continue;
        }
        if (ds) {
          rc = run_conv(h, lds, xin, nullptr, y1, nn, 0, st);
          if (rc) return rc;
          if (upto == lds) { *last = o[1]; return AVVAD_OK; }
          res = y1;
        }
        rc = run_conv(h, lb, y0, res, y2, nn, 1, st);
        if (rc) return rc;
        cur = o[2];
        *last = cur;
        if (upto == lb) return AVVAD_OK;
        layer += ds ? 3 : 2;
      }
    }
  }
  return AVVAD_OK;
}

static int check_loaded(avvad_resnet18* h) {
  for (int i = 0; i < 20; ++i)
    if (!h->set[i]) {
      set_error("resnet18: conv layer " + std::to_string(i) + " not loaded");
      return AVVAD_ERR_STATE;
    }
  return AVVAD_OK;
}

static int forward_common(avvad_resnet18* h, const StemInput& in, int64_t n_frames, int64_t chunk_frames,
                          void* workspace, size_t workspace_bytes, float* feat, void* feat_bf16, int64_t ld_bf16,
                          int64_t col_off, cudaStream_t st) {
  AVVAD_CHECK_ARG(feat || feat_bf16, "at least one output required");
  int rc = check_loaded(h);
  if (rc) return rc;
  if (workspace_bytes < avvad_resnet18_workspace_bytes(n_frames, chunk_frames)) {
    set_error("resnet18: workspace too small");
    return AVVAD_ERR_WORKSPACE;
  }
  const int64_t mc = chunk_of(n_frames, chunk_frames);
  const size_t bsz = align_up((size_t)mc * kActBytesPerFrame, 1024);
  __nv_bfloat16* buf[4];
  for (int i = 0; i < 4; ++i) buf[i] = reinterpret_cast<__nv_bfloat16*>((uint8_t*)workspace + i * bsz);
  for (int64_t f0 = 0; f0 < n_frames; f0 += mc) {
    const int64_t n = (n_frames - f0 < mc) ? (n_frames - f0) : mc;
    int last = 0;
    rc = run_trunk_chunk(h, in.advance(f0), n, buf, 20, &last, st);
    if (rc) return rc;
    const int64_t total = n * (512 / 8);
    avgpool_kernel<<<(unsigned)ceil_div(total, 256), 256, 0, st>>>(
        buf[last], n, 9, 512, feat ? feat + f0 * 512 : nullptr,
        feat_bf16 ? (__nv_bfloat16*)feat_bf16 + f0 * ld_bf16 : nullptr, ld_bf16, col_off);
    AVVAD_LAUNCHED();
  }
  return AVVAD_OK;
}

extern "C" int avvad_resnet18_forward(avvad_resnet18* h, const float* frames, int64_t n_frames, int64_t chunk_frames,
                                      void* workspace, size_t workspace_bytes, float* feat, void* feat_bf16,
                                      int64_t ld_bf16, int64_t col_off, void* stream) {
  AVVAD_CHECK_ARG(h && frames && workspace && n_frames > 0, "bad argument");
  StemInput in;
  in.frames = frames;
  return forward_common(h, in, n_frames, chunk_frames, workspace, workspace_bytes, feat, feat_bf16, ld_bf16, col_off,
                        (cudaStream_t)stream);
}

extern "C" int avvad_resnet18_forward_u8(avvad_resnet18* h, const uint8_t* src, const int32_t* n_src,
                                         const int32_t* n_out, int32_t B, int32_t f_max, int32_t t_max, int32_t num,
                                         int32_t den, float mean, float stdv, float eps, int standardise,
                                         int64_t chunk_frames, void* workspace, size_t workspace_bytes, float* feat,
                                         void* feat_bf16, int64_t ld_bf16, int64_t col_off, void* stream) {
  AVVAD_CHECK_ARG(h && src && n_src && n_out && workspace, "null pointer");
  AVVAD_CHECK_ARG(B > 0 && f_max > 0 && t_max > 0 && num > 0 && den > 0, "non-positive size");
  StemInput in;
  in.src = src; in.n_src = n_src; in.n_out = n_out;
  in.f_max = f_max; in.t_max = t_max; in.num = num; in.den = den;
  in.mean = mean; in.denom = stdv + eps; in.standardise = standardise;
  in.src_bytes = (int64_t)B * f_max * kFrameHW;
  return forward_common(h, in, (int64_t)B * t_max, chunk_frames, workspace, workspace_bytes, feat, feat_bf16, ld_bf16,
                        col_off, (cudaStream_t)stream);
}

extern "C" int avvad_resnet18_forward_upto(avvad_resnet18* h, const float* frames, int64_t n_frames, int upto,
                                           void* workspace, size_t workspace_bytes, void* out_act, void* stream) {
  AVVAD_CHECK_ARG(h && frames && workspace && out_act && n_frames > 0 && upto >= 0 && upto < 20, "bad argument");
  int rc = check_loaded(h);
  if (rc) return rc;
  if (workspace_bytes < avvad_resnet18_workspace_bytes(n_frames, n_frames)) {
    set_error("resnet18: workspace too small (forward_upto runs a single chunk)");
    return AVVAD_ERR_WORKSPACE;
  }
  cudaStream_t st = (cudaStream_t)stream;
  const size_t bsz = align_up((size_t)n_frames * kActBytesPerFrame, 1024);
  __nv_bfloat16* buf[4];
  for (int i = 0; i < 4; ++i) buf[i] = reinterpret_cast<__nv_bfloat16*>((uint8_t*)workspace + i * bsz);
  int last = 0;
  StemInput in;
  in.frames = frames;
  rc = run_trunk_chunk(h, in, n_frames, buf, upto, &last, st);
  if (rc) return rc;
  const ConvSpec& s = kSpecs[upto];
  const int ho = (upto == 0) ? 17 : s.hout;
  const size_t bytes = (size_t)n_frames * ho * ho * s.cout * sizeof(__nv_bfloat16);
  AVVAD_CUDA(cudaMemcpyAsync(out_act, buf[last], bytes, cudaMemcpyDeviceToDevice, st));
  return AVVAD_OK;
}

extern "C" int avvad_resnet18_set_conv_train(avvad_resnet18* h, int layer, const float* w, const float* gamma,
                                             const float* beta, void* stream) {
  AVVAD_CHECK_ARG(h && layer >= 0 && layer < 20 && w && gamma && beta, "bad argument");
  cudaStream_t st = (cudaStream_t)stream;
  const ConvSpec& s = kSpecs[layer];
  const size_t wn = (layer == 0) ? 64 * 64 : (size_t)s.cout * s.cin * s.k * s.k;
  if (!h->wraw[layer]) {
    AVVAD_CUDA(cudaMalloc(&h->wraw[layer], wn * sizeof(__nv_bfloat16)));
    AVVAD_CUDA(cudaMalloc(&h->gamma[layer], s.cout * sizeof(float)));
    AVVAD_CUDA(cudaMalloc(&h->beta[layer], s.cout * sizeof(float)));
  }
  if (layer == 0) {
    if (!h->w1raw32) {
      AVVAD_CUDA(cudaMalloc(&h->w1raw32, 64 * 49 * sizeof(float)));
      AVVAD_CUDA(cudaMalloc(&h->w1fold, 64 * 64 * sizeof(__nv_bfloat16)));
    }
    pack_conv1_raw32_kernel<<<13, 256, 0, st>>>(w, h->w1raw32);
    AVVAD_LAUNCHED();
    pack_conv1_raw_kernel<<<16, 256, 0, st>>>(w, h->wraw[0]);
  } else
    pack_conv_raw_kernel<<<(unsigned)ceil_div((int64_t)wn, 256), 256, 0, st>>>(w, s.cout, s.cin, s.k, h->wraw[layer]);
  AVVAD_LAUNCHED();
  AVVAD_CUDA(cudaMemcpyAsync(h->gamma[layer], gamma, s.cout * sizeof(float), cudaMemcpyDeviceToDevice, st));
  AVVAD_CUDA(cudaMemcpyAsync(h->beta[layer], beta, s.cout * sizeof(float), cudaMemcpyDeviceToDevice, st));
  h->set_train[layer] = true;
  return AVVAD_OK;
}

extern "C" size_t avvad_resnet18_train_workspace_bytes(int64_t n_frames) {
  if (n_frames <= 0) return 0;
  const size_t act = align_up((size_t)n_frames * kActBytesPerFrame, 1024);
  return 5 * act + 64 * 1024;
}

namespace {
struct TrainCtx {
  avvad_resnet18* h;
  int64_t n;
  double* stats;
  float* mean_invstd;
  float bn_eps, momentum;
  float* const* running_mean;
  float* const* running_var;
  cudaStream_t st;
};

int bn_train(const TrainCtx& c, int layer, const __nv_bfloat16* raw, int64_t M, int C, const __nv_bfloat16* residual,
             int relu, __nv_bfloat16* out, float* mean_invstd_out = nullptr) {
  AVVAD_CUDA(cudaMemsetAsync(c.stats, 0, sizeof(double) * 2 * C, c.st));
  const int lanes = 256 / (C / 8);
  bn_stats_kernel<<<(unsigned)ceil_div(M, kStatRows), 256, (size_t)lanes * 2 * C * sizeof(float), c.st>>>(raw, M, C,
                                                                                                        c.stats);
  AVVAD_LAUNCHED();
  bn_finalize_kernel<<<(unsigned)ceil_div(C, 128), 128, 0, c.st>>>(
      c.stats, M, C, c.bn_eps, c.momentum, c.h->gamma[layer], c.h->beta[layer], c.mean_invstd,
      c.running_mean ? c.running_mean[layer] : nullptr, c.running_var ? c.running_var[layer] : nullptr, mean_invstd_out);
  AVVAD_LAUNCHED();
  const int rows_per_block = lanes * kApplyRows;
  bn_apply_kernel<<<(unsigned)ceil_div(M, rows_per_block), 256, 2 * C * sizeof(float), c.st>>>(
      raw, M, C, c.mean_invstd, residual, relu, out);
  AVVAD_LAUNCHED();
  return AVVAD_OK;
}

int conv_raw(const TrainCtx& c, int layer, const __nv_bfloat16* in, __nv_bfloat16* raw) {
  const ConvSpec& s = kSpecs[layer];
  return avvad_conv2d_nhwc_bf16(in, c.h->wraw[layer], nullptr, nullptr, raw, c.n, s.hin, s.hin, s.cin, s.cout, s.k, s.k,
                                s.stride, s.pad, 0, c.st);
}
}

extern "C" int avvad_resnet18_forward_train(avvad_resnet18* h, const float* frames, int64_t n_frames, void* workspace,
                                            size_t workspace_bytes, float bn_eps, float momentum,
                                            float* const* running_mean, float* const* running_var, float* feat,
                                            void* feat_bf16, int64_t ld_bf16, int64_t col_off, void* stream) {
  AVVAD_CHECK_ARG(h && frames && workspace && n_frames > 0 && (feat || feat_bf16), "bad argument");
  for (int i = 0; i < 20; ++i)
    if (!h->set_train[i]) {
      set_error("resnet18: training weights of conv layer " + std::to_string(i) + " not loaded");
      return AVVAD_ERR_STATE;
    }
  if (workspace_bytes < avvad_resnet18_train_workspace_bytes(n_frames)) {
    set_error("resnet18: training workspace too small");
    return AVVAD_ERR_WORKSPACE;
  }
  cudaStream_t st = (cudaStream_t)stream;
  const int64_t n = n_frames;
  const size_t act = align_up((size_t)n * kActBytesPerFrame, 1024);
  uint8_t* p = (uint8_t*)workspace;
  __nv_bfloat16* buf[4];
  for (int i = 0; i < 4; ++i) buf[i] = reinterpret_cast<__nv_bfloat16*>(p + i * act);
  __nv_bfloat16* raw = reinterpret_cast<__nv_bfloat16*>(p + 4 * act);
  double* stats = reinterpret_cast<double*>(p + 5 * act);
  float* mean_invstd = reinterpret_cast<float*>(p + 5 * act + 16 * 1024);
  TrainCtx c{h, n, stats, mean_invstd, bn_eps, momentum, running_mean, running_var, st};

  {
    StemInput sin;
    sin.frames = frames;
    AVVAD_CUDA(cudaMemsetAsync(stats, 0, sizeof(double) * 2 * 64, st));
    int rc = launch_stem_s2d(h, sin, n, nullptr, st, h->wraw[0], nullptr, stats);
    if (rc) return rc;
    bn_finalize_kernel<<<1, 128, 0, st>>>(stats, n * 1156, 64, bn_eps, momentum, h->gamma[0], h->beta[0], mean_invstd,
                                          running_mean ? running_mean[0] : nullptr,
                                          running_var ? running_var[0] : nullptr);
    AVVAD_LAUNCHED();
    fold_conv1_kernel<<<16, 256, 0, st>>>(h->w1raw32, mean_invstd, h->w1fold);
    AVVAD_LAUNCHED();
    rc = launch_stem_s2d(h, sin, n, buf[0], st, h->w1fold, mean_invstd + 64);
    if (rc) return rc;
  }
  int cur = 0, layer = 1;
  for (int stage = 0; stage < 4; ++stage) {
    for (int blk = 0; blk < 2; ++blk) {
      int o[3], k = 0;
      for (int i = 0; i < 4; ++i)
        if (i != cur) o[k++] = i;
      const bool ds = (stage > 0 && blk == 0);
      const int la = layer, lb = layer + 1, lds = layer + 2;
      const ConvSpec& sa = kSpecs[la];
      const int64_t Mo = n * sa.hout * sa.hout;
      int rc = conv_raw(c, la, buf[cur], raw);
      if (rc) return rc;
      rc = bn_train(c, la, raw, Mo, sa.cout, nullptr, 1, buf[o[0]]);
      if (rc) return rc;
      const __nv_bfloat16* res = buf[cur];
      if (ds) {
        rc = conv_raw(c, lds, buf[cur], raw);
        if (rc) return rc;
        rc = bn_train(c, lds, raw, Mo, sa.cout, nullptr, 0, buf[o[1]]);
        if (rc) return rc;
        res = buf[o[1]];
      }
      rc = conv_raw(c, lb, buf[o[0]], raw);
      if (rc) return rc;
      rc = bn_train(c, lb, raw, Mo, sa.cout, res, 1, buf[o[2]]);
      if (rc) return rc;
      cur = o[2];
      layer += ds ? 3 : 2;
    }
  }
  const int64_t total = n * (512 / 8);
  avgpool_kernel<<<(unsigned)ceil_div(total, 256), 256, 0, st>>>(buf[cur], n, 9, 512, feat,
                                                                 (__nv_bfloat16*)feat_bf16, ld_bf16, col_off);
  AVVAD_LAUNCHED();
  return AVVAD_OK;
}

#include "resnet_bwd.cuh"
```

### audio-visual-vad_b200/csrc/stem_s2d.cuh

```cuda
#pragma once
#include "gemm_tc.cuh"

namespace avvad {
namespace tc {

constexpr int kS2Builders = 256;
constexpr int kS2BuilderWarps = kS2Builders / 32;
constexpr int kS2EpiWarps = 8;
constexpr int kS2EpiThreads = kS2EpiWarps * 32;
constexpr int kS2ChPerWarp = 64 / (kS2EpiWarps / 4);
constexpr int kS2Passes = kS2ChPerWarp / 16;
constexpr int kS2Items = (67 * 37 + kS2Builders - 1) / kS2Builders;
constexpr int kS2Threads = kS2Builders + 32 + kS2EpiThreads;
constexpr int kS2FramesPerBatch = 2;
constexpr int kS2RowsPerFrame = 37;
constexpr int kS2Pitch = 160;
constexpr int kS2PlaneRows = 83;
constexpr uint32_t kS2PlaneBytes = kS2PlaneRows * kS2Pitch;
constexpr int kS2EdgeRows = 132;
constexpr uint32_t kS2EdgeChunkBytes = kS2EdgeRows * 16;
constexpr uint32_t kS2EdgePlaneBytes = 2 * kS2EdgeChunkBytes;
constexpr uint32_t kS2BufBytes = 2 * kS2PlaneBytes + 2 * kS2EdgePlaneBytes;
constexpr uint32_t kS2WStepBytes = 256 * 32;
constexpr uint32_t kS2WBytes = 8 * kS2WStepBytes;
constexpr uint32_t kS2OnesBytes = 128 * 32;
constexpr int kS2RingRows = 32;
constexpr uint32_t kS2RingRowBytes = 16 * 128;
constexpr uint32_t kS2RingBytes = kS2RingRows * kS2RingRowBytes;
constexpr uint32_t kS2EdgeHpBytes = 80 * 128;
constexpr uint32_t kS2OffW = 2 * kS2BufBytes;
constexpr uint32_t kS2OffOnes = kS2OffW + kS2WBytes;
constexpr uint32_t kS2OffRing = kS2OffOnes + kS2OnesBytes;
constexpr uint32_t kS2OffEdgeHp = kS2OffRing + kS2RingBytes;
constexpr uint32_t kS2OffLut = kS2OffEdgeHp + kS2EdgeHpBytes;
constexpr uint32_t kS2OffBias = kS2OffLut + 512;
constexpr uint32_t kS2OffBar = kS2OffBias + 256;
constexpr uint32_t kS2StageBytes = 288 * 16;
constexpr uint32_t kS2OffStage = kS2OffBar + 128;
constexpr uint32_t kS2Smem = 1024 + kS2OffStage + 2 * kS2StageBytes;
static_assert(kS2Smem <= 227 * 1024, "stem kernel: shared memory");

struct StemS2Params {
  const float* frames;
  const uint8_t* src;
  const int32_t* n_src;
  const int32_t* n_out;
  int f_max, t_max, num, den;
  float mean, denom;
  int standardise;
  int64_t n_frames;
  int64_t first;
  const __nv_bfloat16* w1b;
  int64_t src_bytes;
  const float* bias;
  __nv_bfloat16* out;
  double* stats;
};

__device__ __forceinline__ uint32_t desc_lo_ns(uint32_t saddr, uint32_t lbo_bytes) {
  return ((saddr & 0x3FFFFu) >> 4) | ((lbo_bytes >> 4) << 16);
}
__device__ __forceinline__ uint32_t desc_hi_ns(uint32_t sbo_bytes) { return (sbo_bytes >> 4) | (1u << 14); }

__device__ __forceinline__ void umma_f16_ns(uint32_t tmem_d, uint32_t a_lo, uint32_t a_hi, uint32_t b_lo, uint32_t b_hi,
                                            uint32_t idesc, uint32_t accum) {
  asm volatile(
      "{\n\t.reg .pred p;\n\t.reg .b64 da, db;\n\t"
      "mov.b64 da, {%1, %2};\n\t"
      "mov.b64 db, {%3, %4};\n\t"
      "setp.ne.b32 p, %6, 0;\n\t"
      "tcgen05.mma.cta_group::1.kind::f16 [%0], da, db, %5, p;\n\t}"
      ::"r"(tmem_d), "r"(a_lo), "r"(a_hi), "r"(b_lo), "r"(b_hi), "r"(idesc), "r"(accum)
      : "memory");
}

__device__ __forceinline__ int s2_src_index(int k, int n_src, int num, int den) {
  long long v = ((long long)den * (2LL * k + 1) - 1) / (2LL * num);
  return v < n_src - 1 ? (int)v : n_src - 1;
}

__device__ __forceinline__ void named_bar_sync(int id, int nthreads) {
  asm volatile("bar.sync %0, %1;" ::"r"(id), "r"(nthreads) : "memory");
}

__device__ __forceinline__ uint32_t bf16x2_max(uint32_t a, uint32_t b) {
  uint32_t r;
  asm("max.bf16x2 %0, %1, %2;" : "=r"(r) : "r"(a), "r"(b));
  return r;
}

template <int MODE, bool STATS = false>
__global__ void __launch_bounds__(kS2Threads, 1) stem_s2d_kernel(const StemS2Params p) {
  extern __shared__ uint8_t smem_raw[];
  const uint32_t raw = smem_u32(smem_raw);
  const uint32_t base = (raw + 1023u) & ~1023u;
  uint8_t* smem = smem_raw + (base - raw);
  float* bias_s = reinterpret_cast<float*>(smem + kS2OffBias);
  unsigned short* lut = reinterpret_cast<unsigned short*>(smem + kS2OffLut);
  const uint32_t bar0 = base + kS2OffBar;
  auto BAR = [&](int i) { return bar0 + 8u * (uint32_t)i; };
  volatile uint32_t* tmem_slot = reinterpret_cast<volatile uint32_t*>(smem + kS2OffBar + 96);

  const int tid = threadIdx.x;
  const int warp = tid >> 5, lane = tid & 31;
  const int64_t n_batches = (p.n_frames + kS2FramesPerBatch - 1) / kS2FramesPerBatch;

  for (uint32_t i = tid; i < (2 * kS2BufBytes) / 16; i += kS2Threads)
    reinterpret_cast<uint4*>(smem)[i] = make_uint4(0u, 0u, 0u, 0u);
  for (int idx = tid; idx < 7 * 256 * 16; idx += kS2Threads) {
    const int e = idx & 15, n = (idx >> 4) & 255, fr = idx >> 12;
    const int s = n >> 6, ch = n & 63;
    const int fs = e - 2 * s;
    __nv_bfloat16 v = __float2bfloat16_rn(0.f);
    if (fs >= 0 && fs < 7) v = p.w1b[ch * 64 + fr * 7 + fs];
    const uint32_t off = kS2OffW + (uint32_t)fr * kS2WStepBytes + (uint32_t)(n >> 3) * 256u + (uint32_t)(e >> 3) * 128u +
                         (uint32_t)(n & 7) * 16u + (uint32_t)(e & 7) * 2u;
    *reinterpret_cast<__nv_bfloat16*>(smem + off) = v;
  }
  for (int idx = tid; idx < 256 * 16; idx += kS2Threads) {
    const int e = idx & 15, n = idx >> 4;
    const float bv = p.bias ? p.bias[n & 63] : 0.f;
    const __nv_bfloat16 hi = __float2bfloat16_rn(bv);
    __nv_bfloat16 v = __float2bfloat16_rn(0.f);
    if (e == 0) v = hi;
    if (e == 1) v = __float2bfloat16_rn(bv - __bfloat162float(hi));
    const uint32_t off = kS2OffW + 7u * kS2WStepBytes + (uint32_t)(n >> 3) * 256u + (uint32_t)(e >> 3) * 128u +
                         (uint32_t)(n & 7) * 16u + (uint32_t)(e & 7) * 2u;
    *reinterpret_cast<__nv_bfloat16*>(smem + off) = v;
  }
  for (uint32_t i = tid; i < kS2OnesBytes / 4; i += kS2Threads)
    reinterpret_cast<uint32_t*>(smem + kS2OffOnes)[i] = 0x3F803F80u;
  if (tid < 64) bias_s[tid] = p.bias ? p.bias[tid] : 0.f;
  if (MODE == 1 && tid < 256) {
    float v = (float)tid;
    if (p.standardise) v = (v - p.mean) / p.denom;
    const __nv_bfloat16 h = __float2bfloat16_rn(v);
    lut[tid] = *reinterpret_cast<const unsigned short*>(&h);
  }
  if (tid == 0) {
    for (int i = 0; i < 2; ++i) {
      mbar_init(BAR(0 + i), kS2Builders);
      mbar_init(BAR(2 + i), 1);
      mbar_init(BAR(4 + i), 1);
      mbar_init(BAR(6 + i), kS2EpiWarps);
    }
    fence_barrier_init();
  }
  if (warp == kS2BuilderWarps) {
    tmem_alloc(smem_u32(const_cast<uint32_t*>(tmem_slot)), 512);
    tmem_relinquish();
  }
  fence_proxy_async();
  tc_fence_before();
  __syncthreads();
  tc_fence_after();
  const uint32_t tmem_acc = *tmem_slot;

  if (warp < kS2BuilderWarps) {
    uint32_t px[MODE == 0 ? kS2Items : 1];
    uint4 ck0 = make_uint4(0u, 0u, 0u, 0u), ck1 = ck0;
    bool live_next = false;
    uint32_t mis_next = 0;
    auto load_chunk = [&](const uint8_t* ptr) -> uint4 {
      if (ptr >= p.src && ptr + 16 <= p.src + p.src_bytes) return __ldg(reinterpret_cast<const uint4*>(ptr));
      uint32_t w[4] = {0u, 0u, 0u, 0u};
      for (int i = 0; i < 16; ++i)
        if (ptr + i >= p.src && ptr + i < p.src + p.src_bytes) w[i >> 2] |= (uint32_t)__ldg(ptr + i) << (8 * (i & 3));
      return make_uint4(w[0], w[1], w[2], w[3]);
    };
    auto fetch = [&](int64_t n) {
      if (MODE == 1) live_next = false;
      if (n >= p.n_frames) return;
      if (MODE == 0) {
        const float* f32 = p.frames + n * (67 * 67);
#pragma unroll
        for (int j = 0; j < kS2Items; ++j) {
          const int item = tid + j * kS2Builders;
          const int r = item / 37, q = item - r * 37;
          const int c0 = 2 * q - 3, c1 = c0 + 1;
          const bool ok0 = (unsigned)c0 < 67u && r < 67, ok1 = (unsigned)c1 < 67u && r < 67;
          const float v0 = ok0 ? __ldg(f32 + r * 67 + c0) : 0.f;
          const float v1 = ok1 ? __ldg(f32 + r * 67 + c1) : 0.f;
          px[j] = pack_bf16x2(v0, v1);
        }
      } else {
        const int64_t ng = p.first + n;
        const int b = (int)(ng / p.t_max), k = (int)(ng - (int64_t)b * p.t_max);
        const int F = p.n_src[b], T = p.n_out[b];
        if (!(k < T && F > 0)) return;
        const uint8_t* u8 = p.src + ((int64_t)b * p.f_max + s2_src_index(k, F, p.num, p.den)) * (67 * 67);
        const uint32_t mis = (uint32_t)(reinterpret_cast<uintptr_t>(u8) & 15u);
        const uint8_t* a0 = u8 - mis;
        live_next = true;
        mis_next = mis;
        ck0 = load_chunk(a0 + 16 * tid);
        if (16u * (uint32_t)(kS2Builders + tid) < 67u * 67u + mis) ck1 = load_chunk(a0 + 16 * (kS2Builders + tid));
      }
    };
    uint32_t stage_sel = 0;
    const uint8_t* sb = nullptr;
    bool live = false;
    auto store = [&]() {
      if (MODE == 1) {
        uint8_t* stage = smem + kS2OffStage + stage_sel * kS2StageBytes;
        stage_sel ^= 1u;
        live = live_next;
        if (live) {
          reinterpret_cast<uint4*>(stage)[tid] = ck0;
          if (kS2Builders + tid < (int)(kS2StageBytes / 16)) reinterpret_cast<uint4*>(stage)[kS2Builders + tid] = ck1;
        }
        sb = stage + mis_next;
      }
    };
    auto build = [&](uint8_t* bufp, int fi) {
#pragma unroll
      for (int j = 0; j < kS2Items; ++j) {
        const int item = tid + j * kS2Builders;
        const int r = item / 37, q = item - r * 37;
        if (r >= 67) continue;
        uint32_t w;
        if (MODE == 0) {
          w = px[j];
        } else {
          const int c0 = 2 * q - 3, c1 = c0 + 1;
          const uint32_t lo = ((unsigned)c0 < 67u) ? (uint32_t)lut[live ? sb[r * 67 + c0] : 0] : 0u;
          const uint32_t hi = ((unsigned)c1 < 67u) ? (uint32_t)lut[live ? sb[r * 67 + c1] : 0] : 0u;
          w = lo | (hi << 16);
        }
        const int pr = r + 3;
        const int yy = fi * kS2RowsPerFrame + (pr >> 1);
        uint8_t* plane = bufp + (uint32_t)(pr & 1) * kS2PlaneBytes;
        *reinterpret_cast<uint32_t*>(plane + yy * kS2Pitch + 4 * q) = w;
        if (q >= 30) {
          uint8_t* edge = bufp + 2 * kS2PlaneBytes + (uint32_t)(pr & 1) * kS2EdgePlaneBytes;
          *reinterpret_cast<uint32_t*>(edge + (uint32_t)((q - 30) >> 2) * kS2EdgeChunkBytes + yy * 16 + 4 * ((q - 30) & 3)) = w;
        }
      }
    };
    uint32_t it = 0;
    fetch((int64_t)blockIdx.x * kS2FramesPerBatch);
    for (int64_t bi = blockIdx.x; bi < n_batches; bi += gridDim.x, ++it) {
      const uint32_t buf = it & 1u;
      mbar_wait(BAR(2 + buf), ((it >> 1) & 1u) ^ 1u);
      uint8_t* bufp = smem + buf * kS2BufBytes;
#pragma unroll
      for (int fi = 0; fi < kS2FramesPerBatch; ++fi) {
        const int64_t n = bi * kS2FramesPerBatch + fi;
        const bool have = n < p.n_frames;
        if (have) store();
        if (MODE == 0 && have) build(bufp, fi);
        const int64_t nn = (fi + 1 < kS2FramesPerBatch) ? n + 1 : (bi + gridDim.x) * kS2FramesPerBatch;
        if (fi + 1 < kS2FramesPerBatch || bi + gridDim.x < n_batches) fetch(nn);
        if (MODE == 1 && have) {
          named_bar_sync(2, kS2Builders);
          build(bufp, fi);
        }
      }
      fence_proxy_async();
      mbar_arrive(BAR(0 + buf));
    }
  } else if (warp == kS2BuilderWarps) {
    constexpr uint32_t idesc = make_idesc(256);
    const uint32_t a_hi_main = desc_hi_ns(kS2Pitch), a_hi_edge = desc_hi_ns(128), b_hi = desc_hi_ns(256);
    uint32_t it = 0, g = 0;
    for (int64_t bi = blockIdx.x; bi < n_batches; bi += gridDim.x, ++it) {
      const uint32_t buf = it & 1u;
      const int nf = (int)((p.n_frames - bi * kS2FramesPerBatch) < kS2FramesPerBatch
                               ? (p.n_frames - bi * kS2FramesPerBatch)
                               : kS2FramesPerBatch);
      const int n_main = (nf * kS2RowsPerFrame + 15) / 16;
      mbar_wait(BAR(0 + buf), (it >> 1) & 1u);
      tc_fence_after();
      const uint32_t bufa = base + buf * kS2BufBytes;
      for (int t = -1; t < n_main; ++t, ++g) {
        const uint32_t acc = g & 1u;
        mbar_wait(BAR(6 + acc), ((g >> 1) & 1u) ^ 1u);
        tc_fence_after();
        if (elect_one_sync()) {
          const uint32_t d = tmem_acc + acc * 256u;
          umma_f16_ns(d, desc_lo_ns(base + kS2OffOnes, 128u), b_hi, desc_lo_ns(base + kS2OffW + 7u * kS2WStepBytes, 128u),
                      b_hi, idesc, 0);
#pragma unroll
          for (int fr = 0; fr < 7; ++fr) {
            const int a = fr >> 1, b = fr & 1;
            uint32_t a_lo, a_hi;
            if (t < 0) {
              a_lo = desc_lo_ns(bufa + 2 * kS2PlaneBytes + (uint32_t)b * kS2EdgePlaneBytes + (uint32_t)a * 16u,
                                kS2EdgeChunkBytes);
              a_hi = a_hi_edge;
            } else {
              a_lo = desc_lo_ns(bufa + (uint32_t)b * kS2PlaneBytes + (uint32_t)(16 * t + a) * kS2Pitch, 16u);
              a_hi = a_hi_main;
            }
            const uint32_t b_lo = desc_lo_ns(base + kS2OffW + (uint32_t)fr * kS2WStepBytes, 128u);
            umma_f16_ns(d, a_lo, a_hi, b_lo, b_hi, idesc, 1);
          }
          umma_commit(BAR(4 + acc));
          if (t == n_main - 1) umma_commit(BAR(2 + buf));
        }
        __syncwarp();
      }
    }
  } else {
    const int ew = warp - (kS2BuilderWarps + 1);
    const int q = warp & 3;
    const int half = ew >> 2;
    const int etid = tid - (kS2Builders + 32);
    const int L = q * 32 + lane;
    uint8_t* ring = smem + kS2OffRing;
    uint8_t* edge_hp = smem + kS2OffEdgeHp;
    uint32_t g = 0;
    if (STATS) {
      float sa[kS2ChPerWarp], sq[kS2ChPerWarp];
#pragma unroll
      for (int c = 0; c < kS2ChPerWarp; ++c) sa[c] = sq[c] = 0.f;
      for (int64_t bi = blockIdx.x; bi < n_batches; bi += gridDim.x) {
        const int nf = (int)((p.n_frames - bi * kS2FramesPerBatch) < kS2FramesPerBatch
                                 ? (p.n_frames - bi * kS2FramesPerBatch)
                                 : kS2FramesPerBatch);
        const int n_rows = nf * kS2RowsPerFrame;
        const int n_main = (n_rows + 15) / 16;
        for (int t = -1; t < n_main; ++t, ++g) {
          const uint32_t acc = g & 1u;
          mbar_wait(BAR(4 + acc), (g >> 1) & 1u);
          tc_fence_after();
          const uint32_t t_row = tmem_acc + acc * 256u + ((uint32_t)(q * 32) << 16);
          const int yy = (t < 0) ? L : 16 * t + (L >> 3);
          const int y = yy % kS2RowsPerFrame;
          const bool live = (yy < n_rows) && (y < 34) && (t >= 0 || L < 80);
          const int s_first = (t < 0) ? 2 : 0;
#pragma unroll 1
          for (int pass = 0; pass < kS2Passes; ++pass) {
            const int ch0 = half * kS2ChPerWarp + pass * 16;
#pragma unroll
            for (int sft = 0; sft < 4; ++sft) {
              uint32_t v[16];
              tmem_ld16(t_row + (uint32_t)sft * 64u + ch0, v);
              tmem_ld_wait();
              if (live && sft >= s_first) {
#pragma unroll
                for (int c = 0; c < 16; ++c) {
                  const float x = __uint_as_float(v[c]);
                  if (kS2Passes == 1 || pass == 0) {
                    sa[c] += x;
                    sq[c] = fmaf(x, x, sq[c]);
                  } else {
                    sa[(16 + c) % kS2ChPerWarp] += x;
                    sq[(16 + c) % kS2ChPerWarp] = fmaf(x, x, sq[(16 + c) % kS2ChPerWarp]);
                  }
                }
              }
            }
          }
          tc_fence_before();
          __syncwarp();
          if (lane == 0) mbar_arrive(BAR(6 + acc));
        }
      }
#pragma unroll
      for (int c = 0; c < kS2ChPerWarp; ++c) {
        float a = sa[c], b = sq[c];
#pragma unroll
        for (int o = 16; o > 0; o >>= 1) {
          a += __shfl_xor_sync(0xffffffffu, a, o);
          b += __shfl_xor_sync(0xffffffffu, b, o);
        }
        if (lane == 0) {
          atomicAdd(p.stats + half * kS2ChPerWarp + c, (double)a);
          atomicAdd(p.stats + 64 + half * kS2ChPerWarp + c, (double)b);
        }
      }
    } else
    for (int64_t bi = blockIdx.x; bi < n_batches; bi += gridDim.x) {
      const int nf = (int)((p.n_frames - bi * kS2FramesPerBatch) < kS2FramesPerBatch
                               ? (p.n_frames - bi * kS2FramesPerBatch)
                               : kS2FramesPerBatch);
      const int n_rows = nf * kS2RowsPerFrame;
      const int n_main = (n_rows + 15) / 16;
      for (int t = -1; t < n_main; ++t, ++g) {
        const uint32_t acc = g & 1u;
        mbar_wait(BAR(4 + acc), (g >> 1) & 1u);
        tc_fence_after();
        const uint32_t t_row = tmem_acc + acc * 256u + ((uint32_t)(q * 32) << 16);
        if (t < 0) {
#pragma unroll 1
          for (int pass = 0; pass < kS2Passes; ++pass) {
            const int ch0 = half * kS2ChPerWarp + pass * 16;
            uint32_t v1[16], v2[16], v3[16];
            tmem_ld16(t_row + 64u + ch0, v1);
            tmem_ld16(t_row + 128u + ch0, v2);
            tmem_ld16(t_row + 192u + ch0, v3);
            tmem_ld_wait();
            if (L < 80) {
              uint32_t o[8];
#pragma unroll
              for (int c = 0; c < 8; ++c) {
                const float x0 = fmaxf(fmaxf(__uint_as_float(v1[2 * c]), __uint_as_float(v2[2 * c])), __uint_as_float(v3[2 * c]));
                const float x1 = fmaxf(fmaxf(__uint_as_float(v1[2 * c + 1]), __uint_as_float(v2[2 * c + 1])),
                                       __uint_as_float(v3[2 * c + 1]));
                o[c] = pack_relu_bf16x2(x0, x1);
              }
              uint8_t* rowp = edge_hp + L * 128;
              const int k0 = ch0 >> 3;
              *reinterpret_cast<uint4*>(rowp + (((k0) ^ (L & 7)) << 4)) = make_uint4(o[0], o[1], o[2], o[3]);
              *reinterpret_cast<uint4*>(rowp + (((k0 + 1) ^ (L & 7)) << 4)) = make_uint4(o[4], o[5], o[6], o[7]);
            }
          }
          tc_fence_before();
          __syncwarp();
          if (lane == 0) mbar_arrive(BAR(6 + acc));
          named_bar_sync(1, kS2EpiThreads);
          continue;
        }
        const int yy = 16 * t + (L >> 3);
        const int i = L & 7;
        uint8_t* rrow = ring + (uint32_t)(yy & (kS2RingRows - 1)) * kS2RingRowBytes;
#pragma unroll 1
        for (int pass = 0; pass < kS2Passes; ++pass) {
          const int ch0 = half * kS2ChPerWarp + pass * 16;
          uint32_t v0[16], v1[16], v2[16], v3[16];
          tmem_ld16(t_row + ch0, v0);
          tmem_ld16(t_row + 64u + ch0, v1);
          tmem_ld16(t_row + 128u + ch0, v2);
          tmem_ld16(t_row + 192u + ch0, v3);
          tmem_ld_wait();
          uint32_t oa[8], ob[8];
#pragma unroll
          for (int c = 0; c < 16; c += 2) {
            float pa[2], pb[2];
#pragma unroll
            for (int h = 0; h < 2; ++h) {
              const float s0 = __uint_as_float(v0[c + h]), s1 = __uint_as_float(v1[c + h]);
              const float s2 = __uint_as_float(v2[c + h]), s3 = __uint_as_float(v3[c + h]);
              float left = __shfl_up_sync(0xffffffffu, s3, 1);
              left = (i == 0) ? s0 : left;
              pa[h] = fmaxf(fmaxf(left, s0), s1);
              pb[h] = fmaxf(fmaxf(s1, s2), s3);
            }
            oa[c >> 1] = pack_relu_bf16x2(pa[0], pa[1]);
            ob[c >> 1] = pack_relu_bf16x2(pb[0], pb[1]);
          }
          if (yy < n_rows) {
            const int k0 = ch0 >> 3;
            uint8_t* pxa = rrow + (2 * i) * 128;
            uint8_t* pxb = pxa + 128;
            *reinterpret_cast<uint4*>(pxa + (((k0) ^ i) << 4)) = make_uint4(oa[0], oa[1], oa[2], oa[3]);
            *reinterpret_cast<uint4*>(pxa + (((k0 + 1) ^ i) << 4)) = make_uint4(oa[4], oa[5], oa[6], oa[7]);
            *reinterpret_cast<uint4*>(pxb + (((k0) ^ i) << 4)) = make_uint4(ob[0], ob[1], ob[2], ob[3]);
            *reinterpret_cast<uint4*>(pxb + (((k0 + 1) ^ i) << 4)) = make_uint4(ob[4], ob[5], ob[6], ob[7]);
          }
        }
        tc_fence_before();
        __syncwarp();
        if (lane == 0) mbar_arrive(BAR(6 + acc));
        named_bar_sync(1, kS2EpiThreads);

        {
          const int ch = etid & 7, rr = (etid >> 3) & 7, pg = etid >> 6;
          int ys = 16 * t + 2 * rr;
          int fi = (ys >= kS2RowsPerFrame) ? 1 : 0;
          int y = ys - fi * kS2RowsPerFrame;
          if ((y & 1) == 0) {
            ++ys; ++y;
            if (y == kS2RowsPerFrame) { y = 0; ++fi; }
          }
          if ((y & 1) && y <= 33 && ys < n_rows && fi < nf) {
            const int ph = y >> 1;
            const uint8_t* r0 = ring + (uint32_t)(ys & (kS2RingRows - 1)) * kS2RingRowBytes;
            const uint8_t* r1 = ring + (uint32_t)((ys - 1) & (kS2RingRows - 1)) * kS2RingRowBytes;
            const uint8_t* r2 = ring + (uint32_t)((ys - 2) & (kS2RingRows - 1)) * kS2RingRowBytes;
            const bool top = (y >= 2);
            __nv_bfloat16* orow = p.out + ((bi * kS2FramesPerBatch + fi) * 17 + ph) * (17 * 64) + ch * 8;
#pragma unroll
            for (int pw = pg; pw < 17; pw += kS2EpiThreads / 64) {
              uint4 a, b, c;
              if (pw < 16) {
                const uint32_t off = (uint32_t)pw * 128u + (uint32_t)((ch ^ (pw >> 1)) << 4);
                a = *reinterpret_cast<const uint4*>(r0 + off);
                b = *reinterpret_cast<const uint4*>(r1 + off);
                c = top ? *reinterpret_cast<const uint4*>(r2 + off) : b;
              } else {
                a = *reinterpret_cast<const uint4*>(edge_hp + ys * 128 + ((ch ^ (ys & 7)) << 4));
                b = *reinterpret_cast<const uint4*>(edge_hp + (ys - 1) * 128 + ((ch ^ ((ys - 1) & 7)) << 4));
                c = top ? *reinterpret_cast<const uint4*>(edge_hp + (ys - 2) * 128 + ((ch ^ ((ys - 2) & 7)) << 4)) : b;
              }
              uint4 m;
              m.x = bf16x2_max(bf16x2_max(a.x, b.x), c.x);
              m.y = bf16x2_max(bf16x2_max(a.y, b.y), c.y);
              m.z = bf16x2_max(bf16x2_max(a.z, b.z), c.z);
              m.w = bf16x2_max(bf16x2_max(a.w, b.w), c.w);
              *reinterpret_cast<uint4*>(orow + pw * 64) = m;
            }
          }
        }
        named_bar_sync(1, kS2EpiThreads);
      }
    }
  }

  tc_fence_before();
  __syncthreads();
  if (warp == kS2BuilderWarps) {
    __syncwarp();
    tmem_dealloc(tmem_acc, 512);
  }
}

}
}
```

Before: 2.147 million.

## Use padded 18x18 activation layout and row-strip ring pipeline in block17 kernel

Stores stage-0 activations in an 18-pitch padded layout so the fused block17 kernel can treat consecutive frames as one contiguous row strip. It now processes 128-row tiles through a 3-slot X ring and a 4-slot Y ring with guard rows, instead of per-frame 19x19 padded slabs. This removes the wasted MMA work on padding rows (361 rows rounded to 384 per frame) and interleaves the two convs' MMAs. Downstream stage-1 convs and the stem are taught the new pitch. The cost is extra zero stores for pad columns, larger workspace, and more complex halo and barrier bookkeeping.

```diff
diff --git a/audio-visual-vad_b200/csrc/conv_block.cuh b/audio-visual-vad_b200/csrc/conv_block.cuh
--- a/audio-visual-vad_b200/csrc/conv_block.cuh
+++ b/audio-visual-vad_b200/csrc/conv_block.cuh
@@ -5,20 +5,28 @@
 namespace tc {
 
 constexpr int kBlkThreads = 320;
-constexpr int kBlkW = 17, kBlkWp = 19;
-constexpr int kBlkRows = kBlkWp * kBlkWp;
-constexpr uint32_t kBlkSlabBytes = 47104;
+constexpr int kBlkPitch = 18;
+constexpr int kBlkFrameRows = kBlkPitch * kBlkPitch;
+constexpr int kBlkHalo = kBlkPitch + 1;
+constexpr int kBlkXRows = 128 + 2 * kBlkHalo;
+constexpr uint32_t kBlkXSlot = 22528;
+constexpr int kBlkGuardRows = 24;
+constexpr uint32_t kBlkGuard = kBlkGuardRows * 128;
+constexpr uint32_t kBlkYSlot = 128 * 128;
 constexpr uint32_t kBlkWTile = 32 * 128;
 constexpr uint32_t kBlkWBytes = 9 * kBlkWTile;
-constexpr uint32_t kBlkOffY = kBlkSlabBytes;
-constexpr uint32_t kBlkOffW = 3 * kBlkSlabBytes;
+constexpr uint32_t kBlkOffY = 3 * kBlkXSlot;
+constexpr uint32_t kBlkOffW = kBlkOffY + 4 * kBlkYSlot + 2 * kBlkGuard;
 constexpr uint32_t kBlkOffBias = kBlkOffW + 2 * kBlkWBytes;
 constexpr uint32_t kBlkOffBar = kBlkOffBias + 512;
 constexpr uint32_t kBlkSmem = 1024 + kBlkOffBar + 256;
+static_assert(kBlkSmem <= 227 * 1024, "block17: shared memory");
+static_assert(kBlkXSlot >= kBlkXRows * 128 && kBlkGuardRows >= kBlkHalo && kBlkGuardRows % 8 == 0, "block17: ring geometry");
 
 struct BlockGeom {
   int64_t n_frames;
-  int n_pairs;
+  int frames_per_cta;
+  int n_blocks;
   const float* bias_a;
   const float* bias_b;
   const __nv_bfloat16* x;
@@ -36,30 +44,37 @@
   const uint32_t raw = smem_u32(smem_raw);
   const uint32_t base = (raw + 1023u) & ~1023u;
   uint8_t* smem = smem_raw + (base - raw);
-  const uint32_t sX = base, sY = base + kBlkOffY, sW = base + kBlkOffW;
+  const uint32_t sX = base, sW = base + kBlkOffW;
+  const uint32_t sY = base + kBlkOffY + kBlkGuard;
   const uint32_t bar0 = base + kBlkOffBar;
-  enum { XF = 0, XE, AF, AE, BF, BE, YF0, YF1, YE0, YE1, WF, NBAR };
+  enum { XF = 0, XE = 3, AF = 6, AE = 8, BF = 10, BE = 12, YF = 14, YE = 18, WF = 22, NBAR };
   auto BAR = [&](int i) { return bar0 + 8u * (uint32_t)i; };
   volatile uint32_t* tmem_slot = reinterpret_cast<volatile uint32_t*>(smem + kBlkOffBar + 8 * (NBAR + 1));
   float* bias_s = reinterpret_cast<float*>(smem + kBlkOffBias);
 
   const int warp = threadIdx.x >> 5, lane = threadIdx.x & 31;
   const uint32_t rank = pair_rank();
-  const int pair = blockIdx.x >> 1;
-  const int64_t per_round = 2ll * g.n_pairs;
-  const int n_iter = (int)((g.n_frames + per_round - 1) / per_round);
+  const int nb = g.n_blocks;
+  const int64_t f_begin = (int64_t)blockIdx.x * g.frames_per_cta;
+  const int64_t f_end = f_begin + g.frames_per_cta < g.n_frames ? f_begin + g.frames_per_cta : g.n_frames;
+  const int64_t row0 = f_begin * kBlkFrameRows;
+  const int strip_rows = f_end > f_begin ? (int)((f_end - f_begin) * kBlkFrameRows) : 0;
 
   if (threadIdx.x == 0) {
-    mbar_init(BAR(XF), 1);
-    mbar_init(BAR(XE), 1);
-    mbar_init(BAR(AF), 1);
-    mbar_init(BAR(AE), 2 * 8);
-    mbar_init(BAR(BF), 1);
-    mbar_init(BAR(BE), 2 * 8);
-    mbar_init(BAR(YF0), 2 * 8);
-    mbar_init(BAR(YF1), 2 * 8);
-    mbar_init(BAR(YE0), 1);
-    mbar_init(BAR(YE1), 1);
+    for (int i = 0; i < 3; ++i) {
+      mbar_init(BAR(XF + i), 1);
+      mbar_init(BAR(XE + i), 1);
+    }
+    for (int i = 0; i < 2; ++i) {
+      mbar_init(BAR(AF + i), 1);
+      mbar_init(BAR(AE + i), 2 * 8);
+      mbar_init(BAR(BF + i), 1);
+      mbar_init(BAR(BE + i), 2 * 8);
+    }
+    for (int i = 0; i < 4; ++i) {
+      mbar_init(BAR(YF + i), 2 * 8);
+      mbar_init(BAR(YE + i), 1);
+    }
     mbar_init(BAR(WF), 1);
     fence_barrier_init();
     tma_prefetch_desc(&maps.x);
@@ -74,16 +89,14 @@
   if (warp == 1) {
     asm volatile("tcgen05.alloc.cta_group::2.sync.aligned.shared::cta.b32 [%0], %1;" ::"r"(
                      smem_u32(const_cast<uint32_t*>(tmem_slot))),
-                 "r"(512)
+                 "r"(256)
                  : "memory");
     asm volatile("tcgen05.relinquish_alloc_permit.cta_group::2.sync.aligned;" ::: "memory");
   }
   for (int i = threadIdx.x; i < 128; i += kBlkThreads)
     bias_s[i] = (i < 64) ? (g.bias_a ? g.bias_a[i] : 0.f) : (g.bias_b ? g.bias_b[i - 64] : 0.f);
-  for (int i = threadIdx.x; i < 2 * 20 * 8; i += kBlkThreads) {
-    const int slab = i / 160, r = i % 160;
-    *reinterpret_cast<uint4*>(smem + kBlkOffY + slab * kBlkSlabBytes + r * 16) = make_uint4(0u, 0u, 0u, 0u);
-  }
+  for (int i = threadIdx.x; i < (int)(kBlkGuard / 16); i += kBlkThreads)
+    *reinterpret_cast<uint4*>(smem + kBlkOffY + i * 16) = make_uint4(0u, 0u, 0u, 0u);
   fence_proxy_async();
   if (warp == 0) mbar_wait(BAR(WF), 0);
   tc_fence_before();
@@ -95,160 +108,156 @@
   auto LBAR = [&](int i) { return bar0_leader + 8u * (uint32_t)i; };
 
   if (warp == 0) {
-    for (int i = 0; i < n_iter; ++i) {
-      mbar_wait(BAR(XE), ((uint32_t)i & 1u) ^ 1u);
+    for (int j = 0; j < nb; ++j) {
+      const uint32_t s = (uint32_t)j % 3u, k = (uint32_t)j / 3u;
+      mbar_wait(BAR(XE + s), (k & 1u) ^ 1u);
       if (elect_one_sync()) {
-        const int64_t f = ((int64_t)i * g.n_pairs + pair) * 2 + rank;
-        if (rank == 0) mbar_arrive_expect_tx(BAR(XF), 2u * kBlkRows * 128u);
-        tma_load_4d_2sm(sX, &maps.x, 0, -1, -1, (int)f, LBAR(XF));
+        if (rank == 0) mbar_arrive_expect_tx(BAR(XF + s), 2u * kBlkXRows * 128u);
+        tma_load_2d_2sm(sX + s * kBlkXSlot, &maps.x, 0, (int)(row0 + (int64_t)j * 128 - kBlkHalo), LBAR(XF + s));
       }
       __syncwarp();
     }
   } else if (warp == 1) {
     if (rank == 0) {
       constexpr uint32_t idesc = make_idesc_m256(64);
-      auto conv = [&](uint32_t slab, uint32_t wbase, uint32_t d0) {
-        const uint32_t slab_lo = desc_lo(slab);
+      for (int i = 0; i < nb + 3; ++i) {
+        const bool has_a = i < nb, has_b = i >= 3;
+        const int j = i - 3;
+        const uint32_t xs = (uint32_t)i % 3u, sa = (uint32_t)i & 1u, sb = (uint32_t)j & 1u;
+        if (has_a) {
+          mbar_wait(BAR(XF + xs), ((uint32_t)i / 3u) & 1u);
+          mbar_wait(BAR(AE + sa), (((uint32_t)i >> 1) & 1u) ^ 1u);
+        }
+        if (has_b) {
+          for (int b = j; b <= j + 1 && b < nb; ++b)
+            mbar_wait(BAR(YF + (b & 3)), ((uint32_t)b >> 2) & 1u);
+          mbar_wait(BAR(BE + sb), (((uint32_t)j >> 1) & 1u) ^ 1u);
+        }
+        tc_fence_after();
+        if (elect_one_sync()) {
+          const uint32_t xa = sX + xs * kBlkXSlot + kBlkHalo * 128, ya = sY + (uint32_t)(j & 3) * kBlkYSlot;
+          const uint32_t da = tmem_acc + 64 * sa, db = tmem_acc + 128 + 64 * sb;
 #pragma unroll 1
-        for (int tap = 0; tap < 9; ++tap) {
-          const uint32_t w_lo = desc_lo(wbase) + (uint32_t)tap * (kBlkWTile >> 4);
-          const int fr = tap / 3, fs = tap - fr * 3;
-          const uint32_t a0 = slab_lo + (uint32_t)(fr * kBlkWp + fs) * 8u;
-#pragma unroll
-          for (int m = 0; m < 3; ++m) {
-            umma2_f16_lo2(d0 + m * 64, a0 + m * 1024u, w_lo, idesc, tap != 0, kDescHi);
-            umma2_f16_lo2(d0 + m * 64, a0 + m * 1024u + 2, w_lo + 2, idesc, 1, kDescHi);
-            umma2_f16_lo2(d0 + m * 64, a0 + m * 1024u + 4, w_lo + 4, idesc, 1, kDescHi);
-            umma2_f16_lo2(d0 + m * 64, a0 + m * 1024u + 6, w_lo + 6, idesc, 1, kDescHi);
-          }
-        }
-      };
-      for (int i = 0; i <= n_iter; ++i) {
-        if (i < n_iter) {
-          mbar_wait(BAR(XF), (uint32_t)i & 1u);
-          mbar_wait(BAR(AE), ((uint32_t)i & 1u) ^ 1u);
-          tc_fence_after();
-          if (elect_one_sync()) {
-            conv(sX, sW, tmem_acc);
-            umma2_commit_mc2(BAR(XE));
-            umma2_commit_mc2(BAR(AF));
-          }
-          __syncwarp();
-        }
-        if (i >= 1) {
-          const uint32_t j = (uint32_t)(i - 1), slot = j & 1u;
-          mbar_wait(BAR(YF0 + slot), (j >> 1) & 1u);
-          mbar_wait(BAR(BE), (j & 1u) ^ 1u);
-          tc_fence_after();
-          if (elect_one_sync()) {
-            conv(sY + slot * kBlkSlabBytes, sW + kBlkWBytes, tmem_acc + 192);
-            umma2_commit_mc2(BAR(YE0 + slot));
-            umma2_commit_mc2(BAR(BF));
-          }
-          __syncwarp();
-        }
+          for (int tap = 0; tap < 9; ++tap) {
+            const int fr = tap / 3, fs = tap - fr * 3;
+            const uint32_t off = (uint32_t)(((fr - 1) * kBlkPitch + fs - 1) * 128);
+            if (has_a) {
+              const uint32_t a_lo = desc_lo(xa + off), w_lo = desc_lo(sW) + (uint32_t)tap * (kBlkWTile >> 4);
+              umma2_f16_lo2(da, a_lo, w_lo, idesc, tap != 0, kDescHi);
+              umma2_f16_lo2(da, a_lo + 2, w_lo + 2, idesc, 1, kDescHi);
+              umma2_f16_lo2(da, a_lo + 4, w_lo + 4, idesc, 1, kDescHi);
+              umma2_f16_lo2(da, a_lo + 6, w_lo + 6, idesc, 1, kDescHi);
+            }
+            if (has_b) {
+              const uint32_t a_lo = desc_lo(ya + off), w_lo = desc_lo(sW + kBlkWBytes) + (uint32_t)tap * (kBlkWTile >> 4);
+              umma2_f16_lo2(db, a_lo, w_lo, idesc, tap != 0, kDescHi);
+              umma2_f16_lo2(db, a_lo + 2, w_lo + 2, idesc, 1, kDescHi);
+              umma2_f16_lo2(db, a_lo + 4, w_lo + 4, idesc, 1, kDescHi);
+              umma2_f16_lo2(db, a_lo + 6, w_lo + 6, idesc, 1, kDescHi);
+            }
+          }
+          if (has_a) {
+            umma2_commit_mc2(BAR(XE + xs));
+            umma2_commit_mc2(BAR(AF + sa));
+          }
+          if (has_b) {
+            if (j >= 1) umma2_commit_mc2(BAR(YE + ((j - 1) & 3)));
+            umma2_commit_mc2(BAR(BF + sb));
+          }
+        }
+        __syncwarp();
       }
     }
   } else {
     const int q = warp & 3;
     const int jh = (warp - 2) >> 2;
-    int loc[3];
-    int yrow[3];
-#pragma unroll
-    for (int m = 0; m < 3; ++m) {
-      const int p = m * 128 + q * 32 + lane;
-      const int y = p / kBlkWp, x = p - y * kBlkWp;
-      loc[m] = (y < kBlkW && x < kBlkW) ? (y * kBlkW + x) * 64 + 32 * jh : -1;
-      const int r = p + kBlkWp + 1;
-      yrow[m] = (r < kBlkRows) ? r : -1;
-    }
+    const int t = q * 32 + lane;
     const float* ba = bias_s + 32 * jh;
     const float* bb = bias_s + 64 + 32 * jh;
     const uint32_t lane_sel = (uint32_t)(q * 32) << 16;
-    for (int i = 0; i <= n_iter; ++i) {
-      if (i < n_iter) {
-        const uint32_t slot = (uint32_t)i & 1u;
-        mbar_wait(BAR(AF), (uint32_t)i & 1u);
-        mbar_wait(BAR(YE0 + slot), (((uint32_t)i >> 1) & 1u) ^ 1u);
+    auto is_pixel = [&](int r) {
+      const int p = r % kBlkFrameRows;
+      return r < strip_rows && p < 17 * kBlkPitch && p % kBlkPitch != 17;
+    };
+    for (int i = 0; i < nb + 3; ++i) {
+      if (i < nb) {
+        const uint32_t s = (uint32_t)i & 1u, k = (uint32_t)i >> 1;
+        const int ys = i & 3;
+        mbar_wait(BAR(AF + s), k & 1u);
+        mbar_wait(BAR(YE + ys), (((uint32_t)i >> 2) & 1u) ^ 1u);
         tc_fence_after();
-        uint8_t* ys = smem + kBlkOffY + slot * kBlkSlabBytes;
-#pragma unroll
-        for (int m = 0; m < 3; ++m) {
-#pragma unroll
-          for (int hc = 0; hc < 2; ++hc) {
-            uint32_t v[16];
-            tmem_ld16(tmem_acc + (uint32_t)(m * 64 + 32 * jh + 16 * hc) + lane_sel, v);
-            tmem_ld_wait();
-            if (m == 2 && hc == 1) {
-              tc_fence_before();
-              __syncwarp();
-              if (lane == 0) pair_arrive(LBAR(AE));
-            }
-            if (yrow[m] >= 0) {
-              const bool valid = loc[m] >= 0;
-              const int r = yrow[m];
-#pragma unroll
-              for (int c = 0; c < 2; ++c) {
-                uint32_t w[4];
-#pragma unroll
-                for (int e = 0; e < 4; ++e) {
-                  const float f0 = __uint_as_float(v[8 * c + 2 * e]) + ba[16 * hc + 8 * c + 2 * e];
-                  const float f1 = __uint_as_float(v[8 * c + 2 * e + 1]) + ba[16 * hc + 8 * c + 2 * e + 1];
-                  w[e] = valid ? pack_relu_bf16x2(f0, f1) : 0u;
-                }
-                const int chunk = (4 * jh + 2 * hc + c) ^ (r & 7);
-                *reinterpret_cast<uint4*>(ys + r * 128 + chunk * 16) = make_uint4(w[0], w[1], w[2], w[3]);
-              }
-            }
+        const bool valid = is_pixel(i * 128 + t);
+        uint8_t* yrow = smem + kBlkOffY + kBlkGuard + ys * kBlkYSlot + t * 128;
+        uint8_t* mrow = nullptr;
+        if (ys == 0 && t < kBlkGuardRows) mrow = smem + kBlkOffY + kBlkGuard + 4 * kBlkYSlot + t * 128;
+        if (ys == 3 && t >= 128 - kBlkGuardRows) mrow = smem + kBlkOffY + (t - (128 - kBlkGuardRows)) * 128;
+#pragma unroll
+        for (int hc = 0; hc < 2; ++hc) {
+          uint32_t v[16];
+          tmem_ld16(tmem_acc + 64 * s + (uint32_t)(32 * jh + 16 * hc) + lane_sel, v);
+          tmem_ld_wait();
+          if (hc == 1) {
+            tc_fence_before();
+            __syncwarp();
+            if (lane == 0) pair_arrive(LBAR(AE + s));
+          }
+#pragma unroll
+          for (int c = 0; c < 2; ++c) {
+            uint32_t w[4];
+#pragma unroll
+            for (int e = 0; e < 4; ++e) {
+              const float f0 = __uint_as_float(v[8 * c + 2 * e]) + ba[16 * hc + 8 * c + 2 * e];
+              const float f1 = __uint_as_float(v[8 * c + 2 * e + 1]) + ba[16 * hc + 8 * c + 2 * e + 1];
+              w[e] = valid ? pack_relu_bf16x2(f0, f1) : 0u;
+            }
+            const int chunk = (4 * jh + 2 * hc + c) ^ (t & 7);
+            const uint4 val = make_uint4(w[0], w[1], w[2], w[3]);
+            *reinterpret_cast<uint4*>(yrow + chunk * 16) = val;
+            if (mrow) *reinterpret_cast<uint4*>(mrow + chunk * 16) = val;
           }
         }
         fence_proxy_async();
         __syncwarp();
-        if (lane == 0) pair_arrive(LBAR(YF0 + slot));
-      }
-      if (i >= 1) {
-        const int j = i - 1;
-        const int64_t f = ((int64_t)j * g.n_pairs + pair) * 2 + rank;
-        const bool live = f < g.n_frames;
-        const int64_t foff = f * (int64_t)(kBlkW * kBlkW * 64);
-        u32x8 rb[3][2] = {};
-#pragma unroll
-        for (int m = 0; m < 3; ++m)
-          if (live && loc[m] >= 0) {
-            rb[m][0] = ld_global_256(g.x + foff + loc[m]);
-            rb[m][1] = ld_global_256(g.x + foff + loc[m] + 16);
-          }
-        mbar_wait(BAR(BF), (uint32_t)j & 1u);
+        if (lane == 0) pair_arrive(LBAR(YF + ys));
+      }
+      if (i >= 3) {
+        const int j = i - 3;
+        const uint32_t s = (uint32_t)j & 1u, k = (uint32_t)j >> 1;
+        const int r = j * 128 + t;
+        const bool store = r < strip_rows;
+        const bool valid = is_pixel(r);
+        const int64_t off = (row0 + r) * 64 + 32 * jh;
+        u32x8 rb[2] = {};
+        if (valid) {
+          rb[0] = ld_global_256(g.x + off);
+          rb[1] = ld_global_256(g.x + off + 16);
+        }
+        mbar_wait(BAR(BF + s), k & 1u);
         tc_fence_after();
 #pragma unroll
-        for (int m = 0; m < 3; ++m)
-#pragma unroll
-          for (int c = 0; c < 2; ++c)
-#pragma unroll
-            for (int e = 0; e < 8; ++e) asm volatile("" : "+r"(rb[m][c].v[e]));
-#pragma unroll
-        for (int m = 0; m < 3; ++m) {
-#pragma unroll
-          for (int c = 0; c < 2; ++c) {
-            uint32_t v[16];
-            tmem_ld16(tmem_acc + 192u + (uint32_t)(m * 64 + 32 * jh + 16 * c) + lane_sel, v);
-            tmem_ld_wait();
-            if (m == 2 && c == 1) {
-              tc_fence_before();
-              __syncwarp();
-              if (lane == 0) pair_arrive(LBAR(BE));
-            }
-            if (live && loc[m] >= 0) {
-              u32x8 o;
-#pragma unroll
-              for (int e = 0; e < 8; ++e) {
-                const uint32_t rw = rb[m][c].v[e];
-                const float f0 = __uint_as_float(v[2 * e]) + bb[16 * c + 2 * e] + __uint_as_float(rw << 16);
-                const float f1 = __uint_as_float(v[2 * e + 1]) + bb[16 * c + 2 * e + 1] + __uint_as_float(rw & 0xFFFF0000u);
-                o.v[e] = pack_relu_bf16x2(f0, f1);
-              }
-              st_global_256(g.z + foff + loc[m] + 16 * c, o);
-            }
+        for (int c = 0; c < 2; ++c)
+#pragma unroll
+          for (int e = 0; e < 8; ++e) asm volatile("" : "+r"(rb[c].v[e]));
+#pragma unroll
+        for (int c = 0; c < 2; ++c) {
+          uint32_t v[16];
+          tmem_ld16(tmem_acc + 128 + 64 * s + (uint32_t)(32 * jh + 16 * c) + lane_sel, v);
+          tmem_ld_wait();
+          if (c == 1) {
+            tc_fence_before();
+            __syncwarp();
+            if (lane == 0) pair_arrive(LBAR(BE + s));
+          }
+          if (store) {
+            u32x8 o;
+#pragma unroll
+            for (int e = 0; e < 8; ++e) {
+              const uint32_t rw = rb[c].v[e];
+              const float f0 = __uint_as_float(v[2 * e]) + bb[16 * c + 2 * e] + __uint_as_float(rw << 16);
+              const float f1 = __uint_as_float(v[2 * e + 1]) + bb[16 * c + 2 * e + 1] + __uint_as_float(rw & 0xFFFF0000u);
+              o.v[e] = valid ? pack_relu_bf16x2(f0, f1) : 0u;
+            }
+            st_global_256(g.z + off + 16 * c, o);
           }
         }
       }
@@ -260,7 +269,7 @@
   pair_sync();
   if (warp == 1) {
     __syncwarp();
-    asm volatile("tcgen05.dealloc.cta_group::2.sync.aligned.b32 %0, %1;" ::"r"(tmem_acc), "r"(512) : "memory");
+    asm volatile("tcgen05.dealloc.cta_group::2.sync.aligned.b32 %0, %1;" ::"r"(tmem_acc), "r"(256) : "memory");
   }
 }
 
diff --git a/audio-visual-vad_b200/csrc/conv_slab.cu b/audio-visual-vad_b200/csrc/conv_slab.cu
--- a/audio-visual-vad_b200/csrc/conv_slab.cu
+++ b/audio-visual-vad_b200/csrc/conv_slab.cu
@@ -14,6 +14,8 @@
 int encode_act_map(CUtensorMap* m, const void* ptr, int Cin, int W, int H, int64_t n, const uint32_t box[4],
                    const uint32_t estr[4]);
 int encode_weight_map(CUtensorMap* m, const void* ptr, uint64_t K, uint64_t N, uint32_t bn);
+int encode_tiled_bf16(CUtensorMap* m, const void* ptr, int rank, const uint64_t* dims, const uint64_t* strides_bytes,
+                      const uint32_t* box);
 
 bool slab_supported(int H, int W, int Cin, int Cout, int R, int S, int stride, int pad) {
   return tma_available() && R == 3 && S == 3 && stride == 1 && pad == 1 && H == W && Cin == 64 && Cout == 64;
@@ -137,25 +139,30 @@
     if (cudaGetDevice(&dev) == cudaSuccess) cudaDeviceGetAttribute(&v, cudaDevAttrMultiProcessorCount, dev);
     return v > 0 ? v : 148;
   }();
+  const int64_t rows = n * kBlkFrameRows;
+  AVVAD_CHECK_ARG(rows + 128 < ((int64_t)1 << 31), "block17: too many frames for 32-bit TMA row coordinates");
   BlockMaps maps;
-  const uint32_t box[4] = {64, (uint32_t)kBlkWp, (uint32_t)kBlkWp, 1};
-  const uint32_t estr[4] = {1, 1, 1, 1};
-  int rc = encode_act_map(&maps.x, x, 64, kBlkW, kBlkW, n, box, estr);
+  const uint64_t dims[2] = {64, (uint64_t)rows};
+  const uint64_t strides[1] = {128};
+  const uint32_t box[2] = {64, (uint32_t)kBlkXRows};
+  int rc = encode_tiled_bf16(&maps.x, x, 2, dims, strides, box);
   if (rc) return rc;
   rc = encode_weight_map(&maps.wa, wa, 576, 64, 32);
   if (rc) return rc;
   rc = encode_weight_map(&maps.wb, wb, 576, 64, 32);
   if (rc) return rc;
+  const int64_t want_pairs = (n + 1) / 2, pairs = num_sms / 2;
+  const int n_pairs = (int)(want_pairs < pairs ? want_pairs : pairs);
   BlockGeom g{};
   g.n_frames = n;
-  const int64_t want = (n + 1) / 2, pairs = num_sms / 2;
-  g.n_pairs = (int)(want < pairs ? want : pairs);
+  g.frames_per_cta = (int)((n + 2 * n_pairs - 1) / (2 * n_pairs));
+  g.n_blocks = (int)ceil_div((int64_t)g.frames_per_cta * kBlkFrameRows, 128);
   g.bias_a = bias_a;
   g.bias_b = bias_b;
   g.x = x;
   g.z = z;
   cudaLaunchConfig_t cfg = {};
-  cfg.gridDim = dim3(2u * (unsigned)g.n_pairs);
+  cfg.gridDim = dim3(2u * (unsigned)n_pairs);
   cfg.blockDim = dim3(kBlkThreads);
   cfg.dynamicSmemBytes = kBlkSmem;
   cfg.stream = st;
@@ -172,7 +179,7 @@
     return AVVAD_ERR_CUDA;
   }
   AVVAD_LAUNCHED();
-  prof_end(st, tok, 0, 2.0 * 2.0 * (double)n * kBlkW * kBlkW * 64.0 * 576.0);
+  prof_end(st, tok, 0, 2.0 * 2.0 * (double)n * 17 * 17 * 64.0 * 576.0);
   return AVVAD_OK;
 }
 
diff --git a/audio-visual-vad_b200/csrc/gemm_tma.cu b/audio-visual-vad_b200/csrc/gemm_tma.cu
--- a/audio-visual-vad_b200/csrc/gemm_tma.cu
+++ b/audio-visual-vad_b200/csrc/gemm_tma.cu
@@ -208,7 +208,7 @@
 
 int launch_tma_conv(const __nv_bfloat16* in, const __nv_bfloat16* w, const EpiParams& ep, int64_t n, int H, int W,
                     int Cin, int Cout, int R, int S, int stride, int pad, int bn_hint, cudaStream_t st, int cat,
-                    double flops_override, const SecondOperand* second) {
+                    double flops_override, const SecondOperand* second, int in_pitch, int64_t in_frame) {
   const int OH = (H + 2 * pad - R) / stride + 1;
   const int OW = (W + 2 * pad - S) / stride + 1;
   const int KE = (Cin % 64 == 0) ? 64 : 16;
@@ -263,7 +263,9 @@
 
   TmaMaps maps;
   const uint64_t dims[4] = {(uint64_t)Cin, (uint64_t)W, (uint64_t)H, (uint64_t)n};
-  const uint64_t strides[3] = {(uint64_t)Cin * 2, (uint64_t)W * Cin * 2, (uint64_t)H * W * Cin * 2};
+  const uint64_t pitch = in_pitch > 0 ? (uint64_t)in_pitch : (uint64_t)W;
+  const uint64_t frame = in_frame > 0 ? (uint64_t)in_frame : (uint64_t)H * W;
+  const uint64_t strides[3] = {(uint64_t)Cin * 2, pitch * Cin * 2, frame * Cin * 2};
   const uint32_t estr[4] = {1, (uint32_t)stride, (uint32_t)stride, 1};
   for (int p = 0; p < 2; ++p) {
     const int hb = g.hb[p], F = g.F[p];
@@ -275,8 +277,9 @@
     if (dual) {
       const int s2 = second->stride2;
       const uint64_t dims2[4] = {(uint64_t)second->Cin2, (uint64_t)second->W2, (uint64_t)second->H2, (uint64_t)n};
-      const uint64_t strides2[3] = {(uint64_t)second->Cin2 * 2, (uint64_t)second->W2 * second->Cin2 * 2,
-                                    (uint64_t)second->H2 * second->W2 * second->Cin2 * 2};
+      const uint64_t pitch2 = second->pitch2 > 0 ? (uint64_t)second->pitch2 : (uint64_t)second->W2;
+      const uint64_t frame2 = second->frame2 > 0 ? (uint64_t)second->frame2 : (uint64_t)second->H2 * second->W2;
+      const uint64_t strides2[3] = {(uint64_t)second->Cin2 * 2, pitch2 * second->Cin2 * 2, frame2 * second->Cin2 * 2};
       const uint32_t estr2[4] = {1, (uint32_t)s2, (uint32_t)s2, 1};
       const uint32_t box2[4] = {64, (uint32_t)((OW - 1) * s2 + 1), (uint32_t)((hb - 1) * s2 + 1), (uint32_t)F};
       rc = encode4(&maps.a2[p], second->in2, dims2, strides2, box2, estr2, false);
diff --git a/audio-visual-vad_b200/csrc/gemm_tma.cuh b/audio-visual-vad_b200/csrc/gemm_tma.cuh
--- a/audio-visual-vad_b200/csrc/gemm_tma.cuh
+++ b/audio-visual-vad_b200/csrc/gemm_tma.cuh
@@ -608,10 +608,13 @@
 struct SecondOperand {
   const __nv_bfloat16* in2 = nullptr;
   int H2 = 0, W2 = 0, Cin2 = 0, stride2 = 1;
+  int pitch2 = 0;
+  int64_t frame2 = 0;
 };
 int launch_tma_conv(const __nv_bfloat16* in, const __nv_bfloat16* w, const EpiParams& ep, int64_t n, int H, int W,
                     int Cin, int Cout, int R, int S, int stride, int pad, int bn_hint, cudaStream_t st, int cat = 0,
-                    double flops_override = 0.0, const SecondOperand* second = nullptr);
+                    double flops_override = 0.0, const SecondOperand* second = nullptr, int in_pitch = 0,
+                    int64_t in_frame = 0);
 int launch_tma_gemm(const __nv_bfloat16* A, int64_t lda, const __nv_bfloat16* Wt, int64_t ldw, int64_t M, int N, int K,
                     const EpiParams& ep, int epi_mode, int bn_hint, cudaStream_t st, int ksplit = 1,
                     int64_t split_stride = 0);
diff --git a/audio-visual-vad_b200/csrc/resnet.cu b/audio-visual-vad_b200/csrc/resnet.cu
--- a/audio-visual-vad_b200/csrc/resnet.cu
+++ b/audio-visual-vad_b200/csrc/resnet.cu
@@ -31,6 +31,7 @@
 };
 constexpr int64_t kFrameHW = 67 * 67;
 constexpr int64_t kActBytesPerFrame = 17 * 17 * 64 * 2;
+constexpr int64_t kTallActBytesPerFrame = 18 * 18 * 64 * 2;
 
 __global__ void pack_conv_kernel(const float* __restrict__ w, const float* __restrict__ gamma,
                                  const float* __restrict__ beta, const float* __restrict__ mean,
@@ -371,7 +372,7 @@
 extern "C" size_t avvad_resnet18_workspace_bytes(int64_t n_frames, int64_t chunk_frames) {
   if (n_frames <= 0) return 0;
   const int64_t mc = chunk_of(n_frames, chunk_frames);
-  return (size_t)(4 * align_up((size_t)mc * kActBytesPerFrame, 1024));
+  return (size_t)(4 * align_up((size_t)mc * kTallActBytesPerFrame, 1024));
 }
 
 static int run_conv(avvad_resnet18* h, int layer, const __nv_bfloat16* in, const __nv_bfloat16* residual,
@@ -397,8 +398,9 @@
   int64_t first = 0;
 };
 
-static int launch_stem_s2d(avvad_resnet18* h, const StemInput& in, int64_t n, __nv_bfloat16* out, cudaStream_t st,
-                           const __nv_bfloat16* w = nullptr, const float* bias = nullptr, double* stats = nullptr) {
+static int launch_stem_s2d(avvad_resnet18* h, const StemInput& in, int64_t n, __nv_bfloat16* out, bool tall,
+                           cudaStream_t st, const __nv_bfloat16* w = nullptr, const float* bias = nullptr,
+                           double* stats = nullptr) {
   static PerDeviceOnce once;
   AVVAD_CUDA(once.run([] {
     cudaError_t e = cudaFuncSetAttribute(tc::stem_s2d_kernel<0>, cudaFuncAttributeMaxDynamicSharedMemorySize, (int)tc::kS2Smem);
@@ -418,6 +420,7 @@
   p.w1b = w ? w : h->w1b;
   p.bias = w ? bias : h->bias[0];
   p.out = out;
+  p.tall = tall ? 1 : 0;
   p.stats = stats;
   const int64_t batches = (n + tc::kS2FramesPerBatch - 1) / tc::kS2FramesPerBatch;
   const unsigned grid = (unsigned)(batches < num_sms ? batches : num_sms);
@@ -441,9 +444,6 @@
   return AVVAD_OK;
 }
 
-static int launch_stem(avvad_resnet18* h, const StemInput& in, int64_t n, __nv_bfloat16* out, cudaStream_t st) {
-  return launch_stem_s2d(h, in, n, out, st);
-}
 
 static const int64_t kStageIn[4] = {17 * 17 * 64, 17 * 17 * 64, 9 * 9 * 128, 5 * 5 * 256};
 static const int64_t kStageOut[4] = {17 * 17 * 64, 9 * 9 * 128, 5 * 5 * 256, 3 * 3 * 512};
@@ -454,6 +454,9 @@
   int frc = build_fused(h, st);
   if (frc) return frc;
   const bool whole = upto < 20;
+  const bool tall = !whole && tc::block17_enabled() &&
+                    ((reinterpret_cast<uintptr_t>(buf[0]) | reinterpret_cast<uintptr_t>(buf[1]) |
+                      reinterpret_cast<uintptr_t>(buf[2]) | reinterpret_cast<uintptr_t>(buf[3])) & 31) == 0;
   int cur = 0;
   *last = cur;
   int layer = 1;
@@ -461,7 +464,7 @@
     {
       const int64_t f0 = 0, nn = n;
       if (stage == 0) {
-        int rc = launch_stem(h, in.advance(f0), nn, buf[0] + f0 * kStageIn[0], st);
+        int rc = launch_stem_s2d(h, in.advance(f0), nn, buf[0] + f0 * kStageIn[0], tall, st);
         if (rc) return rc;
         if (upto == 0) return AVVAD_OK;
       }
@@ -481,8 +484,7 @@
         __nv_bfloat16* y0 = buf[o[0]] + f0 * kStageOut[stage];
         __nv_bfloat16* y1 = buf[o[1]] + f0 * kStageOut[stage];
         __nv_bfloat16* y2 = buf[o[2]] + f0 * kStageOut[stage];
-        if (stage == 0 && !whole && tc::block17_enabled() &&
-            ((reinterpret_cast<uintptr_t>(xin) | reinterpret_cast<uintptr_t>(y2)) & 31) == 0) {
+        if (stage == 0 && tall) {
           int rcb = tc::launch_block17(xin, h->w[la], h->bias[la], h->w[lb], h->bias[lb], y2, nn, st);
           if (rcb) return rcb;
           cur = o[2];
@@ -490,7 +492,19 @@
           layer += 2;
           continue;
         }
-        int rc = run_conv(h, la, xin, nullptr, y0, nn, 1, st);
+        int rc;
+        if (stage == 1 && blk == 0 && tall) {
+          const ConvSpec& s = kSpecs[la];
+          tc::EpiParams ep{};
+          ep.bias = h->bias[la];
+          ep.C = y0;
+          ep.ldc = s.cout;
+          ep.relu = 1;
+          rc = tc::launch_tma_conv(xin, h->w[la], ep, nn, s.hin, s.hin, s.cin, s.cout, s.k, s.k, s.stride, s.pad, 0, st,
+                                   0, 0.0, nullptr, 18, 18 * 18);
+        } else {
+          rc = run_conv(h, la, xin, nullptr, y0, nn, 1, st);
+        }
         if (rc) return rc;
         if (upto == la) { *last = o[0]; return AVVAD_OK; }
         const __nv_bfloat16* res = xin;
@@ -505,6 +519,10 @@
           tc::SecondOperand so;
           so.in2 = xin;
           so.H2 = sd.hin; so.W2 = sd.hin; so.Cin2 = sd.cin; so.stride2 = sd.stride;
+          if (stage == 1 && tall) {
+            so.pitch2 = 18;
+            so.frame2 = 18 * 18;
+          }
           rc = tc::launch_tma_conv(y0, h->wf[stage - 1], ep, nn, sb.hin, sb.hin, sb.cin, sb.cout, sb.k, sb.k, sb.stride,
                                    sb.pad, 0, st, 0, 0.0, &so);
           if (rc) return rc;
@@ -552,7 +570,7 @@
     return AVVAD_ERR_WORKSPACE;
   }
   const int64_t mc = chunk_of(n_frames, chunk_frames);
-  const size_t bsz = align_up((size_t)mc * kActBytesPerFrame, 1024);
+  const size_t bsz = align_up((size_t)mc * kTallActBytesPerFrame, 1024);
   __nv_bfloat16* buf[4];
   for (int i = 0; i < 4; ++i) buf[i] = reinterpret_cast<__nv_bfloat16*>((uint8_t*)workspace + i * bsz);
   for (int64_t f0 = 0; f0 < n_frames; f0 += mc) {
@@ -720,7 +738,7 @@
     StemInput sin;
     sin.frames = frames;
     AVVAD_CUDA(cudaMemsetAsync(stats, 0, sizeof(double) * 2 * 64, st));
-    int rc = launch_stem_s2d(h, sin, n, nullptr, st, h->wraw[0], nullptr, stats);
+    int rc = launch_stem_s2d(h, sin, n, nullptr, false, st, h->wraw[0], nullptr, stats);
     if (rc) return rc;
     bn_finalize_kernel<<<1, 128, 0, st>>>(stats, n * 1156, 64, bn_eps, momentum, h->gamma[0], h->beta[0], mean_invstd,
                                           running_mean ? running_mean[0] : nullptr,
@@ -728,7 +746,7 @@
     AVVAD_LAUNCHED();
     fold_conv1_kernel<<<16, 256, 0, st>>>(h->w1raw32, mean_invstd, h->w1fold);
     AVVAD_LAUNCHED();
-    rc = launch_stem_s2d(h, sin, n, buf[0], st, h->w1fold, mean_invstd + 64);
+    rc = launch_stem_s2d(h, sin, n, buf[0], false, st, h->w1fold, mean_invstd + 64);
     if (rc) return rc;
   }
   int cur = 0, layer = 1;
diff --git a/audio-visual-vad_b200/csrc/stem_s2d.cuh b/audio-visual-vad_b200/csrc/stem_s2d.cuh
--- a/audio-visual-vad_b200/csrc/stem_s2d.cuh
+++ b/audio-visual-vad_b200/csrc/stem_s2d.cuh
@@ -54,6 +54,7 @@
   int64_t src_bytes;
   const float* bias;
   __nv_bfloat16* out;
+  int tall;
   double* stats;
 };
 
@@ -470,7 +471,15 @@
             const uint8_t* r1 = ring + (uint32_t)((ys - 1) & (kS2RingRows - 1)) * kS2RingRowBytes;
             const uint8_t* r2 = ring + (uint32_t)((ys - 2) & (kS2RingRows - 1)) * kS2RingRowBytes;
             const bool top = (y >= 2);
-            __nv_bfloat16* orow = p.out + ((bi * kS2FramesPerBatch + fi) * 17 + ph) * (17 * 64) + ch * 8;
+            const int pitch = p.tall ? 18 : 17;
+            const int64_t frame = bi * kS2FramesPerBatch + fi;
+            __nv_bfloat16* orow = p.out + (frame * (p.tall ? 324 : 289) + ph * pitch) * 64 + ch * 8;
+            if (p.tall) {
+              if (pg == 0) *reinterpret_cast<uint4*>(orow + 17 * 64) = make_uint4(0u, 0u, 0u, 0u);
+              if (ph == 16)
+                for (int pw = pg; pw < 18; pw += kS2EpiThreads / 64)
+                  *reinterpret_cast<uint4*>(orow + (18 + pw) * 64) = make_uint4(0u, 0u, 0u, 0u);
+            }
 #pragma unroll
             for (int pw = pg; pw < 17; pw += kS2EpiThreads / 64) {
               uint4 a, b, c;
```

After: 2.063 million, median of 6. -3.9%, worse.
